# sdrobert/pydrobert-speech

Measured on AMD Instinct MI355X. Metric: frames/s (whole node) + HBM-roofline %, 40-mel fbank 16kHz 25/10ms, higher is better.
Workload: dtype f32

## Files before the change

pydrobert-speech_amd/csrc/pds_internal.h:

```cpp
#pragma once
#include <hip/hip_runtime.h>
#include <stdint.h>

#include <exception>
#include <new>
#include <string>

#include "../../include/pds_amd.h"

namespace pds {

void set_error(const std::string &msg);
int32_t hip_fail(hipError_t err, const char *what);

#define PDS_HIP(call)                                       \
  do {                                                      \
    hipError_t _e = (call);                                 \
    if (_e != hipSuccess) return pds::hip_fail(_e, #call);  \
  } while (0)

struct FastTables {
  int kind = 0;
  int n1 = 0, n2 = 0;
  int rows = 0;
  int num_cus = 0;
  float *d_window = nullptr;
  float *d_twiddle = nullptr;
  float *d_tw_special = nullptr;
  float *d_win_half = nullptr;
  float *d_tw_seed = nullptr;
  float *d_ell_w = nullptr;
  int32_t *d_ell_meta = nullptr;
  int32_t *d_ell_len = nullptr;
  int32_t *d_ell_woff = nullptr;
  int ell_wfloats = 0, ell_slots = 0;
  float *d_seg_w = nullptr;
  int32_t *d_seg_meta = nullptr;
  int seg_rounds = 0, seg_len = 0, seg_wfloats = 0, seg_meta_ints = 0;
  float *d_rs_w = nullptr;
  int32_t *d_rs_meta = nullptr;
  int rs_rounds = 0, rs_len = 0, rs_wfloats = 0;
  float *d_rsn_w = nullptr;
  int32_t *d_rsn_meta = nullptr;
  int rsn_rounds = 0, rsn_len = 0, rsn_wfloats = 0;
  int rs_eslot = -1;
  float *d_ms_w = nullptr;
  int32_t *d_ms_meta = nullptr;
  int ms_rounds = 0, ms_len = 0, ms_wfloats = 0, ms_meta_ints = 0, ms_slots = 0;
  long ms_reads = 0;
  int walk = 0;
  long rs_reads = 0, rs_cost = 0, ell_reads = 0, seg_reads = 0;
  float *d_mf_tab = nullptr;
  int mf_rows = 0;
};

}

struct pds_stft_plan {
  pds_stft_desc d;
  int device = 0;
  int num_bins = 0;
  float *d_window_f32 = nullptr;
  double *d_window_f64 = nullptr;
  int32_t *d_row_ptr = nullptr;
  int32_t *d_col = nullptr;
  float *d_val_f32 = nullptr;
  double *d_val_f64 = nullptr;
  float2 *d_tw_f32 = nullptr;
  double2 *d_tw_f64 = nullptr;
  pds::FastTables fast;
};

namespace pds {
struct SiFftTables {
  int blocks = 0;
  bool big = false;
  float2 *d_spectra = nullptr;
  float2 *d_twiddle = nullptr;
  float2 *d_twiddle2k = nullptr;
  int num_cus = 0;
};
}

struct pds_si_plan {
  pds_si_desc d;
  int device = 0;
  int mpad = 0;
  float *d_taps_f32 = nullptr;
  double *d_taps_f64 = nullptr;
  float *d_window_f32 = nullptr;
  double *d_window_f64 = nullptr;
  pds::SiFftTables fft;
};

namespace pds {

int32_t si_fft_tables_create(pds_si_plan *plan, const double *taps);
void si_fft_tables_destroy(pds_si_plan *plan);
int64_t si_fft_scratch_len(const pds_si_plan *plan, int32_t B, int64_t max_frames);
struct SiFftShape;
SiFftShape si_fft_shape_of(const pds_si_plan *plan, int32_t B, int64_t max_frames);
int32_t launch_si_fft(const pds_si_plan *plan, const float *d_signal, const int64_t *d_offsets,
                      const int64_t *d_lengths, const int64_t *d_nframes, const int64_t *d_row_off,
                      int32_t B, int64_t max_frames, int64_t start, const int64_t *d_starts, float *d_scratch,
                      float *d_out, int64_t out_stride, void *stream);

struct BatchArgs {
  const void *d_signal;
  const int64_t *d_offsets, *d_lengths, *d_nframes, *d_row_off;
  int32_t B;
  int64_t max_frames;
  int32_t pad_left;
  double preemph;
  void *d_out;
  int64_t out_stride;
  hipStream_t stream;
  bool in_f64 = false, out_f64 = false;
  bool in_i16 = false;
  int dl_K = 0;
  double dl_taps[16] = {0};
  int64_t *d_chunk_prefix = nullptr;
  bool stretch = false;
  double *d_stat_part = nullptr;
  int32_t *grid_waves_out = nullptr;
  bool prefix_prepared = false;
};

int32_t launch_stft_generic_f32(const pds_stft_plan *plan, const BatchArgs &a);
int32_t launch_stft_generic_f64(const pds_stft_plan *plan, const BatchArgs &a);
int32_t fast_tables_create(pds_stft_plan *plan, const double *window, const int32_t *row_ptr,
                           const int32_t *col, const double *val);
void fast_tables_destroy(pds_stft_plan *plan);
int32_t launch_stft_fast_f32(const pds_stft_plan *plan, const BatchArgs &a);
void fast_plan_geometry(const pds_stft_plan *plan, int32_t out[3]);
bool fast_has_f64in(const pds_stft_plan *plan);
bool fast_has_fused_deltas(const pds_stft_plan *plan);
bool fast_has_fused_cmvn(const pds_stft_plan *plan);
int32_t launch_chunk_prefix(const int64_t *d_nframes, int B, int groups, int64_t *d_prefix, hipStream_t stream);
int32_t launch_cmvn_rows_partials(const float *d_in, int64_t in_stride, const int64_t *d_row_off, const int64_t *d_nrows,
                                  int32_t B, int32_t C, int32_t norm_var, const int64_t *d_chunk_prefix,
                                  const double *d_partials, int32_t grid_waves, double *d_stats, void *d_out,
                                  int32_t out_is_f64, int64_t out_stride, int32_t *d_zero_var, void *stream);

template <typename F>
int32_t no_throw(const char *what, F &&body) {
  try {
    return body();
  } catch (const std::bad_alloc &) {
    set_error(std::string(what) + ": out of host memory");
    return PDS_ERR_NOMEM;
  } catch (const std::exception &err) {
    set_error(std::string(what) + ": " + err.what());
    return PDS_ERR_INVALID;
  }
}

int32_t check_plan_device(int plan_device, const char *what);

template <typename T>
int32_t upload(T **dst, const T *src, size_t count) {
  *dst = nullptr;
  if (count == 0) return PDS_OK;
  PDS_HIP(hipMalloc((void **)dst, count * sizeof(T)));
  PDS_HIP(hipMemcpy(*dst, src, count * sizeof(T), hipMemcpyHostToDevice));
  return PDS_OK;
}

#ifndef PDS_PREEMPH_FMA
#define PDS_PREEMPH_FMA 1
#endif
__device__ __forceinline__ float preemph_sample(float cur, float prev, float c) {
#if PDS_PREEMPH_FMA
  return fmaf(-c, prev, cur);
#else
  float t;
  asm("v_mul_f32 %0, %1, %2" : "=v"(t) : "v"(c), "v"(prev));
  return cur - t;
#endif
}
__device__ __forceinline__ double preemph_sample(double cur, double prev, double c) {
  double t;
  asm("v_mul_f64 %0, %1, %2" : "=v"(t) : "v"(c), "v"(prev));
  return cur - t;
}

__device__ __forceinline__ int64_t reflect_index(int64_t i, int64_t n) {
  if (i >= 0 && i < n) return i;
  const int64_t period = 2 * n;
  int64_t m = i % period;
  if (m < 0) m += period;
  return m < n ? m : period - 1 - m;
}

}
```

pydrobert-speech_amd/csrc/stft_fast.hip:

```cpp
#include "stft_wave_launch.h"

namespace pds {

#if PDS_STAMPS
unsigned long long *g_stamp_buf = nullptr;
extern "C" __attribute__((visibility("default"))) void pds_debug_set_stamp_buffer(unsigned long long *d_buf) {
  g_stamp_buf = d_buf;
}
#endif

extern "C" __attribute__((visibility("default"))) int32_t pds_build_experiments(void) { return PDS_EXPERIMENTS ? 1 : 0; }

bool fast_has_f64in(const pds_stft_plan *plan) { return plan->fast.kind && fast_f64in_kind(plan->fast.kind); }

static int fast_geometry_rows(const FastTables &ft, int *minw);

bool fast_has_fused_cmvn(const pds_stft_plan *plan) {
  const FastTables &ft = plan->fast;
  int minw = 0;
  if (!ft.kind || ft.n2 != 16 || (ft.n1 != 32 && ft.n1 != 64) || !fast_geometry_rows(ft, &minw)) return false;
  return ft.walk == 1 || ft.walk == 3 || (ft.walk == 2 && minw <= 2);
}

bool fast_has_fused_deltas(const pds_stft_plan *plan) {
  const FastTables &ft = plan->fast;
  return ft.kind && fast_deltas_kind(ft.kind) && ft.rsn_rounds >= 1 && ft.rsn_rounds <= 2 &&
         (!plan->d.include_energy || ft.rs_eslot >= 0);
}

__global__ __launch_bounds__(1024) void chunk_prefix_kernel(const int64_t *nframes, int B, int groups, int64_t *prefix) {
  __shared__ int64_t part[1024];
  const int per = (B + 1023) / 1024, lo = threadIdx.x * per, hi = lo + per < B ? lo + per : B;
  int64_t sum = 0;
  for (int b = lo; b < hi; ++b) sum += (nframes[b] + groups - 1) / groups;
  part[threadIdx.x] = sum;
  __syncthreads();
  for (int step = 1; step < 1024; step <<= 1) {
    const int64_t add = threadIdx.x >= (unsigned)step ? part[threadIdx.x - step] : 0;
    __syncthreads();
    part[threadIdx.x] += add;
    __syncthreads();
  }
  int64_t run = part[threadIdx.x] - sum;
  for (int b = lo; b < hi; ++b) {
    prefix[b] = run;
    run += (nframes[b] + groups - 1) / groups;
  }
  if (threadIdx.x == 1023) prefix[B] = part[1023];
}

int32_t launch_chunk_prefix(const int64_t *d_nframes, int B, int groups, int64_t *d_prefix, hipStream_t stream) {
  hipLaunchKernelGGL(chunk_prefix_kernel, dim3(1), dim3(1024), 0, stream, d_nframes, B, groups, d_prefix);
  PDS_HIP(hipGetLastError());
  return PDS_OK;
}

#define PDS_GEOM(N1, N2, R, MINW) int32_t launch_geom_##N1##_##N2##_##R(const pds_stft_plan *plan, const BatchArgs &a);
#ifdef PDS_DEV_ONLY512
PDS_GEOM(32, 16, 25, 4)
#else
#include "stft_geoms.def"
#endif
#undef PDS_GEOM

static int fast_geometry_rows(const FastTables &ft, int *minw = nullptr) {
  if (!ft.kind) return 0;
#define PDS_GEOM(N1, N2, R, MINW)                          \
  if (ft.n1 == N1 && ft.n2 == N2 && ft.rows <= R) {        \
    if (minw) *minw = MINW;                                \
    return R;                                              \
  }
#ifdef PDS_DEV_ONLY512
  PDS_GEOM(32, 16, 25, 4)
#else
#include "stft_geoms.def"
#endif
#undef PDS_GEOM
  return 0;
}

void fast_plan_geometry(const pds_stft_plan *plan, int32_t out[3]) {
  const FastTables &ft = plan->fast;
  const int rows = fast_geometry_rows(ft);
  out[0] = rows ? ft.n1 : 0;
  out[1] = rows ? ft.n2 : 0;
  out[2] = rows;
}

int32_t launch_stft_fast_f32(const pds_stft_plan *plan, const BatchArgs &a) {
  const FastTables &ft = plan->fast;
  const int rows = fast_geometry_rows(ft);
#define PDS_GEOM(N1, N2, R, MINW) \
  if (ft.n1 == N1 && ft.n2 == N2 && rows == R) return launch_geom_##N1##_##N2##_##R(plan, a);
#ifdef PDS_DEV_ONLY512
  PDS_GEOM(32, 16, 25, 4)
#else
#include "stft_geoms.def"
#endif
#undef PDS_GEOM
  set_error("stft_batch: no fused kernel for this plan");
  return PDS_ERR_INVALID;
}

int32_t fast_tables_create(pds_stft_plan *plan, const double *window, const int32_t *row_ptr,
                           const int32_t *col, const double *val) {
  FastTables &ft = plan->fast;
  ft.kind = 0;
  const pds_stft_desc &d = plan->d;
  int n1 = 0, n2 = 0;
  switch (d.dft_size) {
    case 128: n1 = 16; n2 = 8; break;
    case 256: n1 = 32; n2 = 8; break;
    case 512: n1 = 32; n2 = 16; break;
    case 1024: {
      const char *geom = PDS_EXPERIMENTS ? std::getenv("PDS_N1024_GEOM") : nullptr;
      const bool wide = geom && std::strcmp(geom, "32x32") == 0;
      n1 = wide ? 32 : 64;
      n2 = wide ? 32 : 16;
      break;
    }
    case 2048: n1 = 64; n2 = 32; break;
    case 4096: n1 = 64; n2 = 64; break;
    case 160: n1 = 20; n2 = 8; break;
    case 200: n1 = 25; n2 = 8; break;
    case 240: n1 = 30; n2 = 8; break;
    case 320: n1 = 20; n2 = 16; break;
    case 400: n1 = 25; n2 = 16; break;
    case 480: n1 = 30; n2 = 16; break;
    case 640: n1 = 20; n2 = 32; break;
    case 800: n1 = 25; n2 = 32; break;
    case 960: n1 = 30; n2 = 32; break;
    default: return PDS_OK;
  }
  const bool pow2 = (n1 & (n1 - 1)) == 0;
  if (!pow2 && d.frame_length != d.dft_size) return PDS_OK;
  const char *off = std::getenv("PDS_STFT_GENERIC");
  if (off && off[0] == '1') return PDS_OK;
  if (d.frame_length > d.dft_size || d.frame_length <= d.dft_size / 2) return PDS_OK;
  if (d.frame_shift >= (1 << 22)) return PDS_OK;
  if (d.use_log && !((float)d.log_floor >= 1.17549435e-38f)) return PDS_OK;
  if (d.num_filts > 32767) return PDS_OK;
  const int N = d.dft_size, H1 = n1 / 2, cols = (n1 - 1) / 2 + 1;
  std::vector<float> win((size_t)n1 * n2, 0.0f);
  for (int r = 0; r < n2; ++r)
    for (int k = 0; k < n1; ++k) {
      const int idx = n2 * k + r;
      if (idx < d.frame_length) {
        const float w = (float)window[idx];
        win[(size_t)r * n1 + k] = w == 0.0f ? 0x1p-100f : w;
      }
    }
  std::vector<float> tw((size_t)n2 * cols * 2, 0.0f);
  for (int r = 0; r < n2; ++r)
    for (int k1 = 1; k1 < cols; ++k1) {
      const double ang = -2.0 * M_PI * (double)((r * k1) % N) / (double)N;
      const double scale = (!pow2 || PDS_RDFT_DIT) ? 1.0 : (2 * k1 == H1) ? 1.0 : 0.5;
      tw[((size_t)r * cols + k1) * 2 + 0] = (float)(scale * std::cos(ang));
      tw[((size_t)r * cols + k1) * 2 + 1] = (float)(scale * std::sin(ang));
    }
  std::vector<int32_t> order(d.num_filts);
  for (int f = 0; f < d.num_filts; ++f) order[f] = f;
  auto span = [&](int f) {
    return row_ptr[f + 1] > row_ptr[f] ? col[row_ptr[f + 1] - 1] - (col[row_ptr[f]] & ~3) + 1 : 0;
  };
  std::stable_sort(order.begin(), order.end(), [&](int x, int y) { return span(x) > span(y); });
  const int slots = (d.num_filts + n2 - 1) / n2;
  const int pstr = ((N / 2 + 2 + 15) / 32) * 32 + 16;
  std::vector<int32_t> ell_meta((size_t)std::max(slots, 1) * n2, 0), ell_len(std::max(slots, USLOTS), 0),
      ell_woff(std::max(slots, USLOTS), 0);
  std::vector<float> ell_w;
  for (int sl = 0; sl < slots; ++sl) {
    int longest = 8;
    std::vector<int> first(n2, 0);
    for (int j = 0; j < n2 && sl * n2 + j < d.num_filts; ++j) {
      const int f = order[sl * n2 + j];
      if (row_ptr[f + 1] == row_ptr[f]) continue;
      first[j] = col[row_ptr[f]] & ~3;
      longest = std::max(longest, (span(f) + 7) / 8 * 8);
    }
    {
      std::vector<int> lanes;
      for (int j = 0; j < n2 && sl * n2 + j < d.num_filts; ++j)
        if (span(order[sl * n2 + j]) > 0) lanes.push_back(j);
      std::stable_sort(lanes.begin(), lanes.end(), [&](int x, int y) {
        return span(order[sl * n2 + x]) > span(order[sl * n2 + y]);
      });
      std::vector<std::vector<int>> taken(16);
      for (int j : lanes) {
        const int slack = std::min((longest - span(order[sl * n2 + j])) / 4, first[j] / 4);
        int best_shift = 0, best_cost = 1 << 30;
        for (int sh = 0; sh <= slack; ++sh) {
          const int q = first[j] / 4 - sh;
          int cost = 0;
          for (int other : taken[q % 16]) cost += other != q;
          if (cost < best_cost) {
            best_cost = cost;
            best_shift = sh;
          }
        }
        first[j] -= 4 * best_shift;
        taken[(first[j] / 4) % 16].push_back(first[j] / 4);
      }
    }
    ell_len[sl] = longest;
    ell_woff[sl] = (int32_t)ell_w.size();
    const int wstride = longest + 4;
    ell_w.resize(ell_w.size() + (size_t)n2 * wstride, 0.0f);
    for (int j = 0; j < n2; ++j) {
      const int f = sl * n2 + j < d.num_filts ? order[sl * n2 + j] : -1;
      if (first[j] + longest > pstr)
        first[j] = (pstr - longest) & ~3;
      if (first[j] < 0) return PDS_OK;
      ell_meta[(size_t)sl * n2 + j] = first[j] | ((f + 1) << 16);
      if (f < 0) continue;
      for (int q = row_ptr[f]; q < row_ptr[f + 1]; ++q) {
        const int t = col[q] - first[j];
        if (t < 0 || t >= longest) return PDS_OK;
        ell_w[(size_t)ell_woff[sl] + (size_t)j * wstride + t] = (float)val[q];
      }
    }
  }
  if (ell_w.empty()) ell_w.assign(4, 0.0f);
  ft.ell_wfloats = (int)ell_w.size();
  ft.ell_slots = slots;
  int32_t rc = PDS_OK;
  const int groups = 64 / n2;
  bool dense_bank = false;
  long dense_reads = 0;
  if ((n2 == 16 || (pow2 && n2 >= 32)) && d.num_filts > 0 && d.num_filts <= 65535) {
    long ell_reads = 0;
    for (int sl = 0; sl < slots; ++sl) ell_reads += 2L * (ell_len[sl] / 4);
    ft.ell_reads = ell_reads;
    const int free_slots = (wave_area_floats(n1, n2) - groups * pstr) / groups;
    int best_len = 0, best_rounds = 0;
    long best_reads = 0, any_reads = 0;
    const char *only_len = std::getenv("PDS_SEG_LEN");
    for (int len : {16, 32, 64}) {
      if (only_len && std::atoi(only_len) != len) continue;
      long nseg = 0;
      for (int f = 0; f < d.num_filts; ++f) nseg += (span(f) + len - 1) / len;
      const int rounds = (int)((nseg + 63) / 64);
      if (rounds == 0 || rounds * 64 > 65535) continue;
      int longest = 0;
      for (int f = 0; f < d.num_filts; ++f) longest = std::max(longest, (span(f) + len - 1) / len);
      const long reads = (long)rounds * (len / 4) * (1 + groups) + rounds + (nseg + 63) / 64 + 4 + 4L * ((longest + 3) / 4);
      if (!any_reads || reads < any_reads) any_reads = reads;
      if (rounds * 64 > free_slots) continue;
      if (!best_len || reads < best_reads) best_len = len, best_rounds = rounds, best_reads = reads;
    }
    const char *force = std::getenv("PDS_STFT_SEGMENTED");
    if (!force && std::getenv("PDS_STFT_WALK") && std::strcmp(std::getenv("PDS_STFT_WALK"), "seg") == 0) force = "1";
    auto wanted = [&](long reads) {
      return force      ? force[0] == '1'
             : n2 == 64 ? reads < ell_reads
             : n2 == 32 ? 10 * reads <= 7 * ell_reads
                        : 5 * reads <= 4 * ell_reads || (slots >= 4 && reads < ell_reads);
    };
    const bool want = wanted(best_reads);
    dense_bank = any_reads > 0 && wanted(any_reads);
    dense_reads = any_reads;
    if (best_len && want) {
      const int len = best_len, nslots = best_rounds * 64, wstride = len + 4;
      std::vector<float> seg_w((size_t)nslots * wstride, 0.0f);
      std::vector<int32_t> seg_meta((size_t)nslots + d.num_filts, 0);
      int slot = 0;
      bool ok = true;
      for (int f = 0; f < d.num_filts && ok; ++f) {
        const int count = (span(f) + len - 1) / len;
        seg_meta[(size_t)nslots + f] = slot | (count << 16);
        const int base = count ? col[row_ptr[f]] & ~3 : 0;
        for (int k = 0; k < count; ++k, ++slot) {
          int first = base + k * len;
          if (first + len > pstr) first = (pstr - len) & ~3;
          if (first < 0) ok = false;
          seg_meta[slot] = first;
          for (int q = row_ptr[f]; q < row_ptr[f + 1]; ++q) {
            if (col[q] < base + k * len || col[q] >= base + (k + 1) * len) continue;
            const int t = col[q] - first;
            if (t < 0 || t >= len) ok = false; else seg_w[(size_t)slot * wstride + t] = (float)val[q];
          }
        }
      }
      if (ok) {
        ft.seg_reads = best_reads;
        ft.seg_rounds = best_rounds;
        ft.seg_len = len;
        ft.seg_wfloats = (int)seg_w.size();
        ft.seg_meta_ints = (int)seg_meta.size();
        if (rc == PDS_OK) rc = upload(&ft.d_seg_w, seg_w.data(), seg_w.size());
        if (rc == PDS_OK) rc = upload(&ft.d_seg_meta, seg_meta.data(), seg_meta.size());
      }
    }
  }
  if (n2 == 16 && rc == PDS_OK) {
    RsegTables rs;
    const int area_floats = wave_area_floats(n1, n2);
    if (build_rseg(d.num_filts, row_ptr, col, val, N / 2 + 1, area_floats / 4, 8, rs)) {
      ft.rs_rounds = rs.rounds;
      ft.rs_len = rs.seg_len;
      ft.rs_wfloats = (int)rs.w.size();
      ft.rs_reads = rs.reads_per_lane();
      ft.rs_cost = rs.cost;
      RsegTables rn;
      ft.rs_eslot = -1;
      if (rc == PDS_OK && fast_deltas_kind(N) && build_rseg(d.num_filts, row_ptr, col, val, N / 2 + 1, area_floats / 4, 2, rn, true)) {
        ft.rsn_rounds = rn.rounds;
        ft.rsn_len = rn.seg_len;
        ft.rsn_wfloats = (int)rn.w.size();
        for (size_t at = 0; at < rn.meta.size() && ft.rs_eslot < 0; ++at)
          if ((rn.meta[at] >> 16) == 0) ft.rs_eslot = (int)at;
        rc = upload(&ft.d_rsn_w, rn.w.data(), rn.w.size());
        if (rc == PDS_OK) rc = upload(&ft.d_rsn_meta, rn.meta.data(), rn.meta.size());
      }
      if (rc == PDS_OK) rc = upload(&ft.d_rs_w, rs.w.data(), rs.w.size());
      if (rc == PDS_OK) rc = upload(&ft.d_rs_meta, rs.meta.data(), rs.meta.size());
    }
  }
  if (n2 == 16 && pow2 && rc == PDS_OK && dense_bank) {
    MsegTables ms;
    const int area_floats = wave_area_floats(n1, n2);
    const int max_slots = (area_floats - 4 * pstr) / 16;
    if (build_mseg(d.num_filts, row_ptr, col, val, pstr, max_slots, ms)) {
      ft.ms_rounds = ms.rounds;
      ft.ms_slots = ms.slots;
      ft.ms_len = ms.seg_len;
      ft.ms_wfloats = (int)ms.w.size();
      ft.ms_meta_ints = (int)ms.meta.size();
      ft.ms_reads = ms.reads_per_lane();
      rc = upload(&ft.d_ms_w, ms.w.data(), ms.w.size());
      if (rc == PDS_OK) rc = upload(&ft.d_ms_meta, ms.meta.data(), ms.meta.size());
    }
  }
  {
    const char *force = std::getenv("PDS_STFT_WALK");
    ft.walk = ft.seg_rounds > 0 ? 1 : 0;
    const bool ms_stands_in = ft.walk == 0 && dense_bank && ft.ms_rounds > 0 && N >= PDS_MSEG_MIN_N;
    const long other = ft.walk == 1 ? ft.seg_reads : ms_stands_in ? dense_reads : ft.ell_reads;
    if (ft.rs_rounds > 0 && 10 * ft.rs_reads <= 7 * other) ft.walk = 2;
    if (force && std::strcmp(force, "ell") == 0) ft.walk = 0;
    if (force && std::strcmp(force, "seg") == 0) ft.walk = ft.seg_rounds > 0 ? 1 : 0;
    if (force && std::strcmp(force, "rseg") == 0) ft.walk = ft.rs_rounds > 0 ? 2 : ft.walk;
    if ((ft.walk == 1 || (ft.walk == 0 && ms_stands_in)) && ft.ms_rounds > 0 && N >= PDS_MSEG_MIN_N && !force) ft.walk = 3;
    if (force && std::strcmp(force, "mseg") == 0 && ft.ms_rounds > 0) ft.walk = 3;
    if (std::getenv("PDS_DEBUG_PLAN"))
      std::fprintf(stderr,
                   "pds plan N=%d filters=%d: ell slots %d reads %ld | seg rounds %d len %d reads %ld | rseg rounds %d "
                   "len %d reads %ld cost %ld | mseg rounds %d len %d reads %ld -> walk %d\n",
                   N, d.num_filts, ft.ell_slots, ft.ell_reads, ft.seg_rounds, ft.seg_len, ft.seg_reads, ft.rs_rounds,
                   ft.rs_len, ft.rs_reads, ft.rs_cost, ft.ms_rounds, ft.ms_len, ft.ms_reads, ft.walk);
  }
  if (rc == PDS_OK) rc = upload(&ft.d_ell_w, ell_w.data(), ell_w.size());
  if (rc == PDS_OK) rc = upload(&ft.d_ell_meta, ell_meta.data(), ell_meta.size());
  if (rc == PDS_OK) rc = upload(&ft.d_ell_len, ell_len.data(), ell_len.size());
  if (rc == PDS_OK) rc = upload(&ft.d_ell_woff, ell_woff.data(), ell_woff.size());
  if (rc == PDS_OK) rc = upload(&ft.d_window, win.data(), win.size());
  if (rc == PDS_OK) rc = upload(&ft.d_twiddle, tw.data(), tw.size());
  if (((n1 == 32 || n1 == 64) && n2 == 16) || lean_geometry(n1, n2)) {
    std::vector<float> wh(win), seed((size_t)n2 * 6);
    for (float &v : wh) v *= PDS_RDFT_DIT ? 1.0f : 0.5f;
    const int mult[3] = {1, 4, n1 / 4};
    for (int r = 0; r < n2; ++r)
      for (int j = 0; j < 3; ++j) {
        const double ang = -2.0 * M_PI * (double)((r * mult[j]) % N) / (double)N;
        seed[((size_t)r * 3 + j) * 2 + 0] = (float)std::cos(ang);
        seed[((size_t)r * 3 + j) * 2 + 1] = (float)std::sin(ang);
      }
    if (rc == PDS_OK) rc = upload(&ft.d_win_half, wh.data(), wh.size());
    if (rc == PDS_OK) rc = upload(&ft.d_tw_seed, seed.data(), seed.size());
  }
  std::vector<float> tws((size_t)n2 * 2);
  for (int r = 0; r < n2; ++r) {
    const double ang = -2.0 * M_PI * (double)r / (double)(2 * n2);
    tws[2 * r] = (float)std::cos(ang);
    tws[2 * r + 1] = (float)std::sin(ang);
  }
  if (rc == PDS_OK) rc = upload(&ft.d_tw_special, tws.data(), tws.size());
  {
    const char *front = PDS_EXPERIMENTS ? std::getenv("PDS_STFT_FRONT") : nullptr;
    const int rows = (d.frame_length + n2 - 1) / n2;
    int bucket = 0;
    for (int b : {20, 25, 28, 30, 32})
      if (!bucket && rows <= b) bucket = b;
    MfmaFrontTables mt;
    if (rc == PDS_OK && n1 == 32 && n2 == 16 && bucket && front && std::strcmp(front, "mfma") == 0 &&
        build_mfma_front(n1, bucket, d.frame_length, window, mt)) {
      std::vector<float> image;
      image.reserve(mt.words());
      image.insert(image.end(), mt.win.begin(), mt.win.end());
      for (int32_t v : mt.off) {
        float f;
        std::memcpy(&f, &v, sizeof f);
        image.push_back(f);
      }
      image.insert(image.end(), mt.emask.begin(), mt.emask.end());
      image.insert(image.end(), mt.a_re.begin(), mt.a_re.end());
      image.insert(image.end(), mt.a_im.begin(), mt.a_im.end());
      image.insert(image.end(), mt.tw.begin(), mt.tw.end());
      rc = upload(&ft.d_mf_tab, image.data(), image.size());
      ft.mf_rows = bucket;
    }
  }
  if (rc != PDS_OK) return rc;
  hipDeviceProp_t prop;
  PDS_HIP(hipGetDeviceProperties(&prop, plan->device));
  ft.num_cus = prop.multiProcessorCount;
  ft.n1 = n1;
  ft.n2 = n2;
  ft.rows = (d.frame_length + n2 - 1) / n2;
  ft.kind = d.dft_size;
  return PDS_OK;
}

void fast_tables_destroy(pds_stft_plan *plan) {
  FastTables &ft = plan->fast;
  (void)hipFree(ft.d_window);
  (void)hipFree(ft.d_twiddle);
  (void)hipFree(ft.d_tw_special);
  (void)hipFree(ft.d_win_half);
  (void)hipFree(ft.d_tw_seed);
  (void)hipFree(ft.d_mf_tab);
  (void)hipFree(ft.d_rs_w);
  (void)hipFree(ft.d_ms_w);
  (void)hipFree(ft.d_ms_meta);
  (void)hipFree(ft.d_rsn_w);
  (void)hipFree(ft.d_rsn_meta);
  (void)hipFree(ft.d_rs_meta);
  (void)hipFree(ft.d_seg_w);
  (void)hipFree(ft.d_seg_meta);
  (void)hipFree(ft.d_ell_w);
  (void)hipFree(ft.d_ell_meta);
  (void)hipFree(ft.d_ell_len);
  (void)hipFree(ft.d_ell_woff);
  ft = FastTables();
}

}
```

pydrobert-speech_amd/csrc/stft_wave_kernel.h:

```cpp
#pragma once
#include <algorithm>
#include <atomic>
#include <cmath>
#include <cstdio>
#include <cstdlib>
#include <cstring>
#include <type_traits>
#include <vector>

#include "fft_inlane.h"
#include "mfma_front.h"
#include "rseg_tables.h"
#include "mseg_tables.h"
#include "pds_internal.h"

#include "stft_switches.h"

namespace pds {

__device__ __forceinline__ void keep_alive(float v) { asm volatile("" ::"v"(v)); }

struct FastParams {
  const void *sig;
  const int64_t *offsets, *lengths, *nframes, *row_off;
  void *out;
  int64_t out_stride;
  const float *win_lane;
  const float2 *tw_lane;
  const float2 *tw_special;
  const float *win_half;
  const float2 *tw_seed;
  const float *ell_w;
  const int32_t *ell_meta;
  const int32_t *ell_len;
  const int32_t *ell_woff;
  int ell_wfloats, ell_slots, ell_meta_pad, ell_meta_ints;
  int seg_rounds, seg_len, num_filts;
  int L, S, pad_left, include_energy, use_power, use_log;
  float log_floor, inv_L, preemph;
  double preemph_d;
  int chunks_per_utt, num_utts;
  int waves;
  int area_f;
  unsigned waves_rcp;
  int lds_ticket_off;
  int dyn;
  const float *mf_tab;
  unsigned long long *stamps;
  const int64_t *chunk_prefix;
  double *stat_part;
  int stat_c, stat_cs;
  int lds_stat_off;
  int dl_inner;
  int dl_order;
  int dl_debug;
  int dl_eslot;
  float dl_f1[5], dl_f2[9];
  int step_utts, step_chunks;
};

__device__ __forceinline__ float mul_legacy(float x, float y) {
  float z;
  asm("v_mul_legacy_f32 %0, %1, %2" : "=v"(z) : "v"(x), "v"(y));
  return z;
}

template <int N1>
__device__ __forceinline__ float window_mul(int n1, float x, float w) {
#if PDS_WINDOW_CONTRACT
  return n1 < N1 / 2 ? x * w : mul_legacy(x, w);
#else
  return mul_legacy(x, w);
#endif
}

template <int M>
__device__ __forceinline__ float dpp_row_shr_keep(float old, float src) {
  return __int_as_float(__builtin_amdgcn_update_dpp(__float_as_int(old), __float_as_int(src),
                                                    0x110 + M, 0xf, 0xf, false));
}

__device__ __forceinline__ float fast_log(float x) {
  return __builtin_amdgcn_logf(x) * 0.69314718055994530942f;
}

__device__ __forceinline__ float floor_log(float v, float floor) {
  return fast_log(__builtin_elementwise_maximum(v, floor));
}

typedef int Int4 __attribute__((ext_vector_type(4)));
template <typename T>
__device__ __forceinline__ T load_const(const T *ptr) {
  typedef const T __attribute__((address_space(4))) *const_ptr;
  return *(const_ptr)(uintptr_t)ptr;
}

template <int CTRL>
__device__ __forceinline__ float dpp_add(float x) {
  return x + __int_as_float(__builtin_amdgcn_update_dpp(0, __float_as_int(x), CTRL, 0xf, 0xf, false));
}

__device__ __forceinline__ void wave_sync() {
  __builtin_amdgcn_fence(__ATOMIC_RELEASE, "wavefront");
  __builtin_amdgcn_wave_barrier();
  __builtin_amdgcn_fence(__ATOMIC_ACQUIRE, "wavefront");
}

#ifndef PDS_TWOPASS
#define PDS_TWOPASS 1
#endif
#ifndef PDS_LEAN_2048
#define PDS_LEAN_2048 1
#endif
constexpr bool lean_geometry(int n1, int n2) { return PDS_LEAN_2048 && n1 == 64 && n2 == 32; }
constexpr int wave_area_floats(int n1, int n2) {
  const int cols = (n1 - 1) / 2 + 1, groups = 64 / n2, one_pass = groups * cols * (n2 + 2) * 2;
  return (PDS_TWOPASS && n1 == 64 && n2 == 16) ? 2688 : lean_geometry(n1, n2) ? groups * cols * (n2 + 4) : one_pass;
}
constexpr int win_table_stride(int rows) { return ((rows + 3) & ~3) % 8 == 4 ? ((rows + 3) & ~3) : ((rows + 3) & ~3) + 4; }

template <int N1, int N2, int NROWS>
struct WaveGeom {
  static constexpr int N = N1 * N2;
  static constexpr int NREG = (N1 - 1) / 2;
  static constexpr int COLS = NREG + 1;
  static constexpr int CPL = (COLS + N2 - 1) / N2;
  static constexpr bool FULL = COLS % N2 == 0;
  static constexpr bool DIST = N2 >= 16;
  static constexpr int GROUPS = 64 / N2;
  static constexpr int NB = N / 2 + 1;
  static constexpr int RS = N2 + 2;
  static constexpr bool TWOPASS = PDS_TWOPASS && N1 == 64 && N2 == 16;
  static constexpr bool LEAN = lean_geometry(N1, N2);
  static constexpr int RSF = N2 + 4;
  static constexpr int XROWS = TWOPASS ? N2 : COLS;
  static constexpr int EXCH_F2 = wave_area_floats(N1, N2) / 2;
  static_assert(LEAN ? GROUPS * XROWS * RSF <= EXCH_F2 * 2 : GROUPS * XROWS * RS <= EXCH_F2, "the exchange must fit the wave's area");
  static_assert(!LEAN || (CPL == 1 && N2 >= 32), "lean form: one column per lane");
  static constexpr int PSTR = ((NB + 1 + 15) / 32) * 32 + 16;
  static_assert(GROUPS * PSTR <= EXCH_F2 * 2, "P must fit over the exchange area");
  static constexpr int XMIN_F = LEAN ? GROUPS * XROWS * RSF : GROUPS * XROWS * RS * 2;
  static constexpr int GCH = XMIN_F / 64 < NROWS ? XMIN_F / 64 : NROWS;
  static_assert(N % 2 == 0 && CPL >= 1 && N2 <= 64 && (RS * 8) % 16 == 0, "geometry");
  static_assert(inl::is_pow2(N1) ? (FULL || N2 == 2 * COLS) : 600 % N1 == 0,
                "in-lane DFT sizes: 2^k, or a divisor of 600");
  static_assert(NROWS <= N1 && NROWS > 0, "rows");
};

constexpr int USLOTS = 4;

typedef float f32x4 __attribute__((ext_vector_type(4)));

template <int N1, int N2, int NROWS, int MAXWAVES, int MINW, bool ELL_LDS, bool PRE, int SEG = 0, int MF = 0,
          bool RSG = false, typename TIN = float, typename TOUT = float, int DLT = 0, bool STR = false, bool PF = false>
__global__ __launch_bounds__(MAXWAVES * 64, MINW) void stft_wave_kernel(const FastParams p) {
  static_assert(!PF || (DLT == 0 && !STR && MF == 0 && !PRE && std::is_same<TIN, float>::value && (N1 == 32 || N1 == 64) && N2 == 16),
                "prefetch: 16-lane power-of-two geometries, float32 samples, round-robin scheduling");
  constexpr bool STRETCH = DLT > 0 || STR;
  static_assert(!(STR && DLT > 0), "stretch scheduling is part of the fused-deltas launches already");
  static_assert(DLT == 0 || (DLT == 2 && N2 == 16 && RSG && std::is_same<TOUT, float>::value && MF == 0),
                "fused deltas: row-segment walk, float32 features");
  static_assert(MF == 0 || std::is_same<TIN, float>::value, "matrix-pipe front end: float32 samples");
  static_assert(std::is_same<TIN, float>::value || std::is_same<TIN, double>::value || std::is_same<TIN, int16_t>::value, "samples: float32, float64 or int16");
  using G = WaveGeom<N1, N2, NROWS>;
  constexpr int N = G::N, COLS = G::COLS, NREG = G::NREG, RS = G::RS, NB = G::NB, PSTR = G::PSTR;
  constexpr int MSLOTS = 2 * MF + 1;
  static_assert(MF == 0 || (N2 == 16 && N1 == 32 && MF == mfma_front_steps(NROWS)), "matrix-pipe front end: 32 x 16");
  static_assert(MF == 0 || 4 * MSLOTS * 64 <= G::EXCH_F2 * 2, "edge-frame gather reuses the exchange area");
  constexpr int NBP = (NB + 3) / 4 * 4;
  static_assert(!RSG || (G::GROUPS == 4 && ELL_LDS && !SEG && (NBP + 1) * 4 <= G::EXCH_F2 * 2),
                "row-segment walk: four frames per wave, tables in LDS");
  extern __shared__ __attribute__((aligned(16))) float smem[];
  const int lane = threadIdx.x & 63;
  const int wave = __builtin_amdgcn_readfirstlane(threadIdx.x >> 6);
  const int g = lane / N2, r = lane % N2;
  constexpr bool F64S = std::is_same<TIN, double>::value;
  constexpr bool PAIR = F64S && N2 == 16 && MF == 0;
  const int rho = PAIR ? ((r & 7) * 2 + (r >> 3)) : r;
  constexpr int LOADSPAN = PAIR ? (NROWS + 1) / 2 * 32 : NROWS * N2;
  [[maybe_unused]] const unsigned long long st_entry = PDS_STAMPS ? __builtin_readcyclecounter() : 0;
  float *wbase = smem + wave * p.area_f;
  [[maybe_unused]] double *wstat = reinterpret_cast<double *>(smem + p.lds_stat_off) + wave * (2 * p.stat_cs);
  constexpr bool STATS = STR && G::GROUPS == 4 && (SEG != 0 || (RSG && MINW <= 2));
  [[maybe_unused]] const bool stats_on = STATS && p.stat_part != nullptr;
  [[maybe_unused]] auto stat_add4 = [&](const int col, const float (&v)[4], const int nf) {
    double t1 = 0.0, t2 = 0.0;
#pragma unroll
    for (int q = 0; q < 4; ++q)
      if (q < nf) {
        const double d = (double)v[q];
        t1 += d;
        t2 = fma(d, d, t2);
      }
    wstat[col] += t1;
    wstat[p.stat_cs + col] += t2;
  };
  float2 *exch = reinterpret_cast<float2 *>(wbase) + g * G::XROWS * RS;
  [[maybe_unused]] float *xf = wbase + g * (G::XROWS * G::RSF);
  float *Pg = wbase + g * PSTR;
  const int nthreads = p.waves * 64;
  float2 *sw_lds = reinterpret_cast<float2 *>(smem + p.waves * p.area_f);
  int *meta_lds = reinterpret_cast<int *>(sw_lds + N2);
  float *ellw_lds = reinterpret_cast<float *>(meta_lds + p.ell_meta_pad);
  constexpr bool TWCHAIN = (PF && PDS_PF_TW == 1) || (PAIR && (N1 == 32 || N1 == 64)) || (PDS_DLT_CHAIN && DLT > 0 && N1 == 32 && N2 == 16) || G::LEAN ||
                           (N1 == 64 && N2 == 16 && (SEG == 2 || PDS_LEAN_1024));
  constexpr bool WINLDS = PF && PDS_PF_WIN == 1;
  constexpr bool WINUSE = G::LEAN || (N1 == 64 && N2 == 16 && (SEG == 2 || PDS_LEAN_1024));
  constexpr int WSTR = win_table_stride(NROWS);
  [[maybe_unused]] float *win_lds = ellw_lds + (ELL_LDS ? p.ell_wfloats : 0);
  if constexpr (WINLDS || WINUSE) {
    const float *wsrc = TWCHAIN ? p.win_half : p.win_lane;
    for (int i = threadIdx.x; i < N2 * WSTR; i += p.waves * 64) {
      const int rr = i / WSTR, k = i - rr * WSTR;
      win_lds[i] = k < NROWS ? wsrc[rr * N1 + k] : 0.0f;
    }
  }
  if (threadIdx.x < N2) sw_lds[threadIdx.x] = p.tw_special[threadIdx.x];
  constexpr bool DYN = PDS_DYN && !STRETCH && !PF;
  [[maybe_unused]] int *ticket_lds = reinterpret_cast<int *>(smem + p.lds_ticket_off);
  if constexpr (DYN) {
    if (threadIdx.x == 0) *ticket_lds = p.waves;
  }
  if constexpr (STR && G::GROUPS == 4 && (SEG != 0 || (RSG && MINW <= 2))) {
    if (p.stat_part) {
      double *z = reinterpret_cast<double *>(smem + p.lds_stat_off);
      for (int i = threadIdx.x; i < p.waves * 2 * p.stat_cs; i += p.waves * 64) z[i] = 0.0;
    }
  }
  if constexpr (RSG) {
    int4 *rec_lds = reinterpret_cast<int4 *>(meta_lds);
    for (int i = threadIdx.x; i < p.seg_rounds * 64; i += nthreads) {
      const int m = p.ell_meta[i], f = (m >> 16) - 1;
      rec_lds[i] = make_int4((m & 0x3fff) * 16, __float_as_int((m & (1 << 14)) ? 1.0f : 0.0f),
                             __float_as_int((m & (1 << 15)) ? 1.0f : 0.0f),
                             f >= 0 ? ((p.include_energy ? 1 : 0) + f) * (int)sizeof(TOUT) : -1);
    }
  } else {
    for (int i = threadIdx.x; i < p.ell_meta_pad; i += nthreads)
      meta_lds[i] = i < p.ell_meta_ints ? p.ell_meta[i] : 0;
  }
#if PDS_FAST_PROLOGUE
  static_assert((G::EXCH_F2 * 2) % 4 == 0, "wave areas are zeroed 16 bytes at a time");
  if constexpr (ELL_LDS) {
    const float4 *src4 = reinterpret_cast<const float4 *>(p.ell_w);
    float4 *dst4 = reinterpret_cast<float4 *>(ellw_lds);
    for (int i = threadIdx.x; i < (p.ell_wfloats >> 2); i += nthreads) dst4[i] = src4[i];
  }
  {
    float4 *z4 = reinterpret_cast<float4 *>(smem);
    for (int i = threadIdx.x; i < p.waves * (p.area_f / 4); i += nthreads) z4[i] = make_float4(0.0f, 0.0f, 0.0f, 0.0f);
  }
#else
  if constexpr (ELL_LDS)
    for (int i = threadIdx.x; i < p.ell_wfloats; i += nthreads) ellw_lds[i] = p.ell_w[i];
  for (int i = threadIdx.x; i < p.waves * p.area_f; i += nthreads) smem[i] = 0.0f;
#endif
  __syncthreads();

  [[maybe_unused]] float win[(MF || WINLDS || WINUSE) ? 1 : NROWS];
  [[maybe_unused]] float twr[(MF || TWCHAIN) ? 1 : COLS], twi[(MF || TWCHAIN) ? 1 : COLS];
  [[maybe_unused]] float sd[6] = {0.0f, 0.0f, 0.0f, 0.0f, 0.0f, 0.0f};
  [[maybe_unused]] float mwin[MSLOTS], mare[MF + 1], maim[MF + 1], mtwr[4], mtwi[4];
  [[maybe_unused]] unsigned moff[MSLOTS];
  if constexpr (MF > 0) {
    const float *tab = p.mf_tab;
#pragma unroll
    for (int sl = 0; sl < MSLOTS; ++sl) {
      mwin[sl] = tab[sl * 64 + lane];
      moff[sl] = (unsigned)reinterpret_cast<const int *>(tab)[(MSLOTS + sl) * 64 + lane] * 4u;
    }
#pragma unroll
    for (int t = 0; t <= MF; ++t) {
      mare[t] = tab[(3 * MSLOTS + t) * 64 + lane];
      maim[t] = tab[(3 * MSLOTS + MF + 1 + t) * 64 + lane];
    }
#pragma unroll
    for (int v = 0; v < 4; ++v) {
      const float2 t = reinterpret_cast<const float2 *>(tab + (3 * MSLOTS + 2 * (MF + 1)) * 64)[v * 64 + lane];
      mtwr[v] = t.x;
      mtwi[v] = t.y;
    }
  } else {
    if constexpr (!WINLDS && !WINUSE) {
      const float *wsrc = TWCHAIN ? p.win_half : p.win_lane;
#pragma unroll
      for (int n1 = 0; n1 < NROWS; ++n1) win[n1] = wsrc[rho * N1 + n1];
    }
    if constexpr (TWCHAIN) {
#pragma unroll
      for (int j = 0; j < 3; ++j) {
        const float2 t = p.tw_seed[rho * 3 + j];
        sd[2 * j] = t.x;
        sd[2 * j + 1] = t.y;
      }
    } else {
#pragma unroll
      for (int k1 = 1; k1 <= NREG; ++k1) {
        const float2 t = p.tw_lane[rho * COLS + k1];
        twr[k1] = t.x;
        twi[k1] = t.y;
      }
    }
  }
  [[maybe_unused]] float pfv[PF ? NROWS : 1];
  [[maybe_unused]] float wl[WINLDS ? NROWS : 1];
  [[maybe_unused]] auto read_window = [&]() {
    if constexpr (WINLDS) {
      const float4 *w4 = reinterpret_cast<const float4 *>(win_lds + rho * WSTR);
#pragma unroll
      for (int j = 0; j < (NROWS + 3) / 4; ++j) {
        const float4 w = w4[j];
        const float wv[4] = {w.x, w.y, w.z, w.w};
#pragma unroll
        for (int u = 0; u < 4; ++u)
          if (4 * j + u < NROWS) wl[4 * j + u] = wv[u];
      }
    }
  };
  read_window();
  [[maybe_unused]] bool pf_ready = false;
  [[maybe_unused]] const int pf_lane = __mul24(g, p.S) + r;
  const int L = p.L, S = p.S;
  const bool use_power = p.use_power != 0;
  const int col0 = p.include_energy ? 1 : 0;

  int b = 0;
  int wg = blockIdx.x;
#ifndef PDS_NO_XCD_MAP
  if ((gridDim.x & 7) == 0) wg = (wg & 7) * (gridDim.x >> 3) + (wg >> 3);
#endif
  int chunk = wg * p.waves + wave;
  if constexpr (!STRETCH) {
    while (chunk >= p.chunks_per_utt && b < p.num_utts) {
      chunk -= p.chunks_per_utt;
      ++b;
    }
  }
  [[maybe_unused]] int rnd = 0, rb = 0, rc = wg * p.waves;
  if constexpr (DYN) {
    while (rc >= p.chunks_per_utt && rb < p.num_utts) {
      rc -= p.chunks_per_utt;
      ++rb;
    }
  }
  [[maybe_unused]] auto take_ticket = [&](const int t) {
    const int jn = (int)__umulhi((unsigned)t, p.waves_rcp), o = t - jn * p.waves;
    while (rnd < jn && rb < p.num_utts) {
      rc += p.step_chunks;
      rb += p.step_utts;
      if (rc >= p.chunks_per_utt) {
        rc -= p.chunks_per_utt;
        ++rb;
      }
      ++rnd;
    }
    b = rb;
    chunk = rc + o;
    while (chunk >= p.chunks_per_utt && b < p.num_utts) {
      chunk -= p.chunks_per_utt;
      ++b;
    }
  };
  [[maybe_unused]] int ticket_v = 0;
  [[maybe_unused]] auto fetch_ticket = [&]() {
    if (lane == 0) ticket_v = __hip_atomic_fetch_add(ticket_lds, 1, __ATOMIC_RELAXED, __HIP_MEMORY_SCOPE_WORKGROUP);
  };
  [[maybe_unused]] auto next_item_dyn = [&](int &nfr_, int &n_, int64_t &sig_off_, int64_t &out_row_) {
    const int last_b = b;
    take_ticket(__builtin_amdgcn_readfirstlane(ticket_v));
    const int pb_ = b < p.num_utts ? b : last_b;
    nfr_ = (int)load_const(p.nframes + pb_);
    n_ = (int)load_const(p.lengths + pb_);
    sig_off_ = load_const(p.offsets + pb_);
    out_row_ = load_const(p.row_off + pb_);
  };
  int nfr = 0, n = 0;
  int64_t sig_off = 0, out_row = 0;
  if (!STRETCH && b < p.num_utts) {
    nfr = (int)load_const(p.nframes + b);
    n = (int)load_const(p.lengths + b);
    sig_off = load_const(p.offsets + b);
    out_row = load_const(p.row_off + b);
  }
  constexpr int DR = 2;
  [[maybe_unused]] int left = 0, e_lo = 0, e_hi = 0, c_last = -1;
  [[maybe_unused]] bool piece_open = false, ran = false;
  [[maybe_unused]] float Wp[DR][4], Wc[DR][4], e_keep = 0.0f;
  if constexpr (STRETCH) {
    const int gw = wg * p.waves + wave, GW = (int)gridDim.x * p.waves;
    const int total = (int)load_const(p.chunk_prefix + p.num_utts);
    const int per = total / GW, rem = total - per * GW;
    const int pos = gw * per + (gw < rem ? gw : rem);
    left = per + (gw < rem ? 1 : 0);
    int lo = 0, hi = p.num_utts;
    while (left > 0 && hi - lo > 1) {
      const int mid = (lo + hi) >> 1;
      if ((int)load_const(p.chunk_prefix + mid) <= pos) lo = mid; else hi = mid;
    }
    b = lo;
    e_lo = left > 0 ? pos - (int)load_const(p.chunk_prefix + lo) : 0;
    chunk = 0;
#pragma unroll
    for (int rd = 0; rd < DR; ++rd)
#pragma unroll
      for (int q = 0; q < 4; ++q) Wp[rd][q] = Wc[rd][q] = 0.0f;
  }
  [[maybe_unused]] auto emit_rows = [&](const int ce, const float (&nx)[DR][4]) {
    if (p.dl_debug & 2) return;
    const int C = p.dl_inner;
    const int W = (p.dl_order + 1) * C, WS = (W + 3) & ~3;
    float *stage = wbase;
    wave_sync();
#pragma unroll
    for (int rd = 0; rd < DR; ++rd) {
      if (rd >= p.seg_rounds) break;
      const int cb = reinterpret_cast<const int4 *>(meta_lds)[rd * 64 + lane].w;
      const int col = cb >= 0 ? cb >> 2 : (p.dl_eslot == rd * 64 + lane ? 0 : -1);
      const float v[12] = {Wp[rd][0], Wp[rd][1], Wp[rd][2], Wp[rd][3], Wc[rd][0], Wc[rd][1],
                           Wc[rd][2], Wc[rd][3], nx[rd][0], nx[rd][1], nx[rd][2], nx[rd][3]};
      float *mine = stage + (col >= 0 ? col : 4 * WS + lane);
      const int wrow = col >= 0 ? WS : 0, wk = col >= 0 ? C : 0;
#pragma unroll
      for (int q = 0; q < 4; ++q) {
        float d = p.dl_f1[0] * v[q + 2];
#pragma unroll
        for (int t = 1; t < 5; ++t) d = fmaf(p.dl_f1[t], v[q + 2 + t], d);
        mine[q * wrow] = v[4 + q];
        mine[q * wrow + wk] = d;
        if (p.dl_order == 2) {
          float dd = p.dl_f2[0] * v[q];
#pragma unroll
          for (int t = 1; t < 9; ++t) dd = fmaf(p.dl_f2[t], v[q + t], dd);
          mine[q * wrow + 2 * wk] = dd;
        }
      }
    }
    wave_sync();
    if (!(p.dl_debug & 1)) {
      float *orow = static_cast<float *>(p.out) + (out_row + (int64_t)ce * 4) * p.out_stride;
      const int fh = nfr - ce * 4;
      const int full = W >> 2, tail = W & 3;
      typedef float F4 __attribute__((ext_vector_type(4), aligned(4)));
      if (fh >= 4 && full <= 64) {
        const int l = lane < full ? lane : full - 1;
        float4 val[4];
#pragma unroll
        for (int q = 0; q < 4; ++q) val[q] = *reinterpret_cast<const float4 *>(stage + q * WS + 4 * l);
        if (lane < full) {
#pragma unroll
          for (int q = 0; q < 4; ++q) {
            F4 o = {val[q].x, val[q].y, val[q].z, val[q].w};
            *reinterpret_cast<F4 *>(orow + (int64_t)q * p.out_stride + 4 * l) = o;
          }
        }
      } else {
        for (int l0 = 0; l0 < full; l0 += 64) {
          const int l = l0 + lane;
          if (l < full) {
#pragma unroll 1
            for (int q = 0; q < 4; ++q)
              if (q < fh) {
                const float4 val = *reinterpret_cast<const float4 *>(stage + q * WS + 4 * l);
                F4 o = {val.x, val.y, val.z, val.w};
                *reinterpret_cast<F4 *>(orow + (int64_t)q * p.out_stride + 4 * l) = o;
              }
          }
        }
      }
      if (tail) {
        const int q = tail == 1 ? lane : tail == 2 ? lane >> 1 : (lane * 11) >> 5;
        const int jj = lane - q * tail;
        if (q < fh && q < 4) orow[(int64_t)q * p.out_stride + 4 * full + jj] = stage[q * WS + 4 * full + jj];
      }
    }
    wave_sync();
  };
  [[maybe_unused]] unsigned long long st_acc[8] = {0, 0, 0, 0, 0, 0, 0, 0};
  [[maybe_unused]] unsigned long long st_prev = PDS_STAMPS ? __builtin_readcyclecounter() : 0;
  [[maybe_unused]] const unsigned long long st_loop = st_prev;
  while (STRETCH || b < p.num_utts) {
    if constexpr (STRETCH) {
      if (!piece_open) {
        if (left <= 0) break;
        nfr = (int)load_const(p.nframes + b);
        const int chunks_b = (nfr + G::GROUPS - 1) / G::GROUPS;
        if (e_lo >= chunks_b) {
          ++b;
          e_lo = 0;
          continue;
        }
        n = (int)load_const(p.lengths + b);
        sig_off = load_const(p.offsets + b);
        out_row = load_const(p.row_off + b);
        e_hi = e_lo + left < chunks_b ? e_lo + left : chunks_b;
        c_last = DLT > 0 ? (e_hi < chunks_b ? e_hi : chunks_b - 1) : e_hi - 1;
        chunk = DLT > 0 ? (e_lo > 0 ? e_lo - 1 : 0) : e_lo;
        piece_open = true;
        ran = false;
      }
      if constexpr (STR) {
        if (ran) ++chunk;
        ran = true;
      }
      if (chunk > c_last) {
        if (DLT > 0 && c_last < e_hi) {
          float nx[DR][4];
#pragma unroll
          for (int rd = 0; rd < DR; ++rd)
#pragma unroll
            for (int q = 0; q < 4; ++q) nx[rd][q] = Wc[rd][3];
          emit_rows(c_last, nx);
        }
        if constexpr (STATS) {
          if (stats_on) {
            wave_sync();
            double *dst = p.stat_part + ((int64_t)(wg * p.waves + wave) + b) * (2 * p.stat_c);
            for (int c = lane; c < p.stat_c; c += 64) {
              dst[c] = wstat[c];
              dst[p.stat_c + c] = wstat[p.stat_cs + c];
              wstat[c] = 0.0;
              wstat[p.stat_cs + c] = 0.0;
            }
            wave_sync();
          }
        }
        left -= e_hi - e_lo;
        ++b;
        e_lo = 0;
        piece_open = false;
        continue;
      }
    }
    int nchunk = chunk + p.step_chunks, nb = b + p.step_utts;
    if (nchunk >= p.chunks_per_utt) {
      nchunk -= p.chunks_per_utt;
      ++nb;
    }
    const int pb = nb < p.num_utts ? nb : b;
    const int tb = chunk * G::GROUPS;
    if constexpr (DYN) {
      if (p.dyn) fetch_ticket();
    }
    if (!STRETCH && tb >= nfr) {
      if (DYN && p.dyn) {
        next_item_dyn(nfr, n, sig_off, out_row);
        continue;
      }
      b = nb;
      chunk = nchunk;
      nfr = (int)load_const(p.nframes + pb);
      n = (int)load_const(p.lengths + pb);
      sig_off = load_const(p.offsets + pb);
      out_row = load_const(p.row_off + pb);
      continue;
    }
    PDS_STAMP(7, 0);
    if constexpr (PDS_STAMPS != 0) ++st_acc[6];
    PDS_PHASE(0);
    [[maybe_unused]] int nfr_nx = 0, n_nx = 0;
    [[maybe_unused]] int64_t sig_off_nx = 0, out_row_nx = 0;
    [[maybe_unused]] auto fetch_next_record = [&]() {
      __builtin_amdgcn_sched_barrier(0);
      nfr_nx = (int)load_const(p.nframes + pb);
      n_nx = (int)load_const(p.lengths + pb);
      sig_off_nx = load_const(p.offsets + pb);
      out_row_nx = load_const(p.row_off + pb);
    };
    [[maybe_unused]] auto issue_prefetch = [&]() {
      const int tb2 = nchunk * G::GROUPS, s02 = tb2 * S - p.pad_left;
      pf_ready = nb < p.num_utts && tb2 + G::GROUPS <= nfr_nx && s02 >= 0 && s02 + (G::GROUPS - 1) * S + LOADSPAN <= n_nx;
      const float *base = pf_ready ? static_cast<const float *>(p.sig) + (sig_off_nx + s02) : p.win_lane;
      const float *xp2 = base + (pf_ready ? pf_lane : r);
#pragma unroll
      for (int n1 = 0; n1 < NROWS; ++n1) {
        pfv[n1] = xp2[n1 * N2];
#if PDS_PF_ILV > 0
        __builtin_amdgcn_sched_group_barrier(0x020, 1, 0);
        __builtin_amdgcn_sched_group_barrier(0x002, PDS_PF_ILV, 0);
#endif
      }
    };
    const TIN *x = static_cast<const TIN *>(p.sig) + sig_off;
    const int start0 = tb * S - p.pad_left;
    bool valid = true;
    float energy = 0.0f;
    const float2 sw = sw_lds[r];
    [[maybe_unused]] float even_sum, odd_sum, Ar[COLS], Ai[COLS];
    if constexpr (MF > 0) {
      int fstart[4];
#pragma unroll
      for (int fg = 0; fg < 4; ++fg) fstart[fg] = start0 + fg * S;
      int wmode = 0;
      if (!(tb + 4 <= nfr && start0 >= (PRE ? 1 : 0) && start0 + 3 * S + NROWS * 16 <= n)) {
        valid = tb + g < nfr;
#pragma unroll
        for (int fg = 0; fg < 4; ++fg) {
          const int st = (tb + fg < nfr ? tb + fg : nfr - 1) * S - p.pad_left;
          fstart[fg] = st;
          int mode = (st < (PRE ? 1 : 0) || st + NROWS * 16 > n) ? 1 : 0;
          if (st < -n || st + L > 2 * n) mode = 2;
          wmode = mode > wmode ? mode : wmode;
        }
      }
      float xs[4][MSLOTS];
      if (wmode == 0) {
#pragma unroll
        for (int fg = 0; fg < 4; ++fg) {
          const char *xg = reinterpret_cast<const char *>(reinterpret_cast<const float *>(x) + fstart[fg]);
#pragma unroll
          for (int sl = 0; sl < MSLOTS; ++sl) {
            float v = (PDS_ABLATE & 1) ? (float)(lane + sl) : *reinterpret_cast<const float *>(xg + moff[sl]);
            if constexpr (PRE) v = preemph_sample(v, *reinterpret_cast<const float *>(xg + moff[sl] - 4), p.preemph);
            xs[fg][sl] = v;
          }
        }
      } else {
        float *tmp = wbase;
        const int *offs = reinterpret_cast<const int *>(p.mf_tab) + MSLOTS * 64 + lane;
#pragma unroll 1
        for (int fg = 0; fg < 4; ++fg) {
          const int st = fstart[fg];
#pragma unroll 1
          for (int sl = 0; sl < MSLOTS; ++sl) {
            int i = st + offs[sl * 64];
            if (wmode == 1) {
              i = i < 0 ? -1 - i : (i >= n ? 2 * n - 1 - i : i);
            } else {
              i = (int)reflect_index((int64_t)i, (int64_t)n);
            }
            float v = (float)x[i];
            if (PRE && i > 0) v = preemph_sample(v, (float)x[i - 1], p.preemph);
            tmp[(fg * MSLOTS + sl) * 64 + lane] = v;
          }
        }
        wave_sync();
#pragma unroll
        for (int fg = 0; fg < 4; ++fg)
#pragma unroll
          for (int sl = 0; sl < MSLOTS; ++sl) xs[fg][sl] = tmp[(fg * MSLOTS + sl) * 64 + lane];
        wave_sync();
      }
      if (p.include_energy) {
        const float *em = p.mf_tab + 2 * MSLOTS * 64 + lane;
        float eg[4] = {0.0f, 0.0f, 0.0f, 0.0f};
#pragma unroll
        for (int sl = 0; sl < MSLOTS; ++sl) {
          const float m = em[sl * 64];
#pragma unroll
          for (int fg = 0; fg < 4; ++fg) {
            const float xm = mul_legacy(xs[fg][sl], m);
            eg[fg] = fmaf(xm, xm, eg[fg]);
          }
        }
#pragma unroll
        for (int fg = 0; fg < 4; ++fg) {
          float e = eg[fg];
          e = dpp_add<0xB1>(e);
          e = dpp_add<0x4E>(e);
          e = dpp_add<0x141>(e);
          e = dpp_add<0x140>(e);
          const int ei = __float_as_int(e);
          const float tot = (__int_as_float(__builtin_amdgcn_readlane(ei, 0)) +
                             __int_as_float(__builtin_amdgcn_readlane(ei, 16))) +
                            (__int_as_float(__builtin_amdgcn_readlane(ei, 32)) +
                             __int_as_float(__builtin_amdgcn_readlane(ei, 48)));
          if (g == fg) energy = tot;
        }
      }
      PDS_STAMP(0, 0);
      PDS_STAMP(1, 1);
      PDS_PHASE(4);
      float sv[4][MF], dv[4][MF], cv[4], uv[4];
#pragma unroll
      for (int fg = 0; fg < 4; ++fg) {
        cv[fg] = xs[fg][2 * MF] * mwin[2 * MF];
        float u = cv[fg];
#pragma unroll
        for (int t = 0; t < MF; ++t) {
          const float a = xs[fg][2 * t] * mwin[2 * t];
          sv[fg][t] = fmaf(xs[fg][2 * t + 1], mwin[2 * t + 1], a);
          dv[fg][t] = fmaf(-xs[fg][2 * t + 1], mwin[2 * t + 1], a);
          u += sv[fg][t];
        }
        uv[fg] = u;
      }
      f32x4 accR[4], accI[4];
#pragma unroll
      for (int fg = 0; fg < 4; ++fg) {
        accR[fg] = f32x4{0.0f, 0.0f, 0.0f, 0.0f};
        accI[fg] = f32x4{0.0f, 0.0f, 0.0f, 0.0f};
      }
      if constexpr (!(PDS_ABLATE & 2)) {
#pragma unroll
        for (int t = 0; t < MF; ++t)
#pragma unroll
          for (int fg = 0; fg < 4; ++fg) {
            accR[fg] = __builtin_amdgcn_mfma_f32_16x16x4f32(mare[t], sv[fg][t], accR[fg], 0, 0, 0);
            accI[fg] = __builtin_amdgcn_mfma_f32_16x16x4f32(maim[t], dv[fg][t], accI[fg], 0, 0, 0);
          }
#pragma unroll
        for (int fg = 0; fg < 4; ++fg) {
          accR[fg] = __builtin_amdgcn_mfma_f32_16x16x4f32(mare[MF], cv[fg], accR[fg], 0, 0, 0);
          accI[fg] = __builtin_amdgcn_mfma_f32_16x16x4f32(maim[MF], uv[fg], accI[fg], 0, 0, 0);
        }
      } else {
#pragma unroll
        for (int fg = 0; fg < 4; ++fg) {
          accR[fg] = f32x4{sv[fg][0], sv[fg][1], sv[fg][2], cv[fg]};
          accI[fg] = f32x4{dv[fg][0], dv[fg][1], dv[fg][2], uv[fg]};
        }
      }
      PDS_PHASE(1);
      float2 *mine = reinterpret_cast<float2 *>(wbase) + (4 * g + 1) * RS + r;
      float *row0 = wbase + r;
#pragma unroll
      for (int fg = 0; fg < 4; ++fg) {
#pragma unroll
        for (int v = 0; v < 4; ++v) {
          float2 val;
          val.x = accR[fg][v] * mtwr[v] - accI[fg][v] * mtwi[v];
          val.y = accR[fg][v] * mtwi[v] + accI[fg][v] * mtwr[v];
          if (v < 3 || g != 3) {
            mine[fg * COLS * RS + v * RS] = val;
          } else {
            row0[fg * COLS * RS * 2] = accR[fg][3];
            row0[fg * COLS * RS * 2 + 16] = accI[fg][3];
          }
        }
      }
    } else {
      int start = start0 + __mul24(g, S);
      int wmode = 0;
      if (!(PF && pf_ready) && !(tb + G::GROUPS <= nfr && start0 >= (PRE ? 1 : 0) &&
            start0 + (G::GROUPS - 1) * S + LOADSPAN <= n)) {
        valid = tb + g < nfr;
        start = (valid ? tb + g : nfr - 1) * S - p.pad_left;
        int mode = 0;
        if (start < (PRE ? 1 : 0) || start + LOADSPAN > n) mode = 1;
        if (start < -n || start + L > 2 * n) mode = 2;
        wmode = __builtin_amdgcn_readfirstlane(__any(mode == 2) ? 2 : (__any(mode == 1) ? 1 : 0));
      }

      float a[N1];
      if (PF && pf_ready) {
#pragma unroll
        for (int n1 = 0; n1 < NROWS; ++n1) a[n1] = pfv[n1];
      } else if (wmode == 0) {
        const TIN *xp = x + (start + r);
        if constexpr (PAIR) {
          typedef double D2 __attribute__((ext_vector_type(2), aligned(8)));
          const TIN *xq = x + (start + 2 * r);
          constexpr int NP = (NROWS + 1) / 2;
          D2 w2[NP];
          [[maybe_unused]] double before = 0.0;
#pragma unroll
          for (int j = 0; j < NP; ++j) w2[j] = *reinterpret_cast<const D2 *>(xq + 32 * j);
          if constexpr (PRE) {
            if (r == 0) before = xq[-1];
          }
          [[maybe_unused]] auto dpp64 = [](double old, double src, auto ctrl) {
            const long long o = __double_as_longlong(old), s_ = __double_as_longlong(src);
            const int lo = __builtin_amdgcn_update_dpp((int)o, (int)s_, decltype(ctrl)::value, 0xf, 0xf, false);
            const int hi = __builtin_amdgcn_update_dpp((int)(o >> 32), (int)(s_ >> 32), decltype(ctrl)::value, 0xf, 0xf, false);
            return __longlong_as_double(((long long)hi << 32) | (unsigned)lo);
          };
#pragma unroll
          for (int j = 0; j < NP; ++j) {
            double u = w2[j].x, v = w2[j].y;
            if constexpr (PRE) {
              const double wrap = j == 0 ? before : dpp64(0.0, (double)w2[j > 0 ? j - 1 : 0].y, inl::Int<0x121>{});
              const double pu = dpp64(wrap, (double)w2[j].y, inl::Int<0x111>{});
              v = preemph_sample(w2[j].y, w2[j].x, (TIN)p.preemph_d);
              u = preemph_sample(w2[j].x, pu, (TIN)p.preemph_d);
            }
            const float fu = (float)u, fv = (float)v;
            a[2 * j] = __int_as_float(__builtin_amdgcn_update_dpp(__float_as_int(fu), __float_as_int(fv), 0x128, 0xf, 0xc, false));
            if (2 * j + 1 < NROWS)
              a[2 * j + 1] = __int_as_float(__builtin_amdgcn_update_dpp(__float_as_int(fv), __float_as_int(fu), 0x128, 0xf, 0x3, false));
          }
        } else if constexpr (F64S) {
          constexpr int FB = (PRE && PDS_F64_ROW_BATCH > 0) ? PDS_F64_ROW_BATCH / 2 : NROWS;
#pragma unroll
          for (int n0 = 0; n0 < NROWS; n0 += FB) {
            TIN cur[FB], prev[FB];
#pragma unroll
            for (int i = 0; i < FB; ++i) {
              if (n0 + i < NROWS) {
                cur[i] = xp[(n0 + i) * N2];
                if constexpr (PRE) prev[i] = xp[(n0 + i) * N2 - 1];
              }
            }
            if constexpr (PRE && PDS_F64_ROW_BATCH > 0) __builtin_amdgcn_sched_barrier(0);
#pragma unroll
            for (int i = 0; i < FB; ++i) {
              if (n0 + i < NROWS) {
                TIN v = cur[i];
                if constexpr (PRE) v = preemph_sample(v, prev[i], (TIN)p.preemph_d);
                a[n0 + i] = (float)v;
              }
            }
          }
        } else {
#pragma unroll
        for (int n1 = 0; n1 < NROWS; ++n1) a[n1] = (PDS_ABLATE & 1) ? (float)(lane + n1) : (float)xp[n1 * N2];
        }
        if constexpr (PRE && !F64S) {
          if constexpr (N2 == 16) {
#if PDS_PREEMPH_DPP
            float carry = 0.0f;
            if (r == 0) carry = (float)xp[-1];
            const float negc = -p.preemph;
            inl::static_for<0, NROWS>([&](auto k) {
              constexpr int n1 = NROWS - 1 - decltype(k)::value;
              if constexpr (n1 > 0) {
                if constexpr (std::is_same<TIN, float>::value)
                  asm volatile("v_fmac_f32_dpp %0, %0, %2 row_shr:1 row_mask:0xf bank_mask:0xf\n\t"
                               "v_fmac_f32_dpp %0, %1, %2 row_shl:15 row_mask:0xf bank_mask:0xf"
                               : "+v"(a[n1]) : "v"(a[n1 - 1]), "v"(negc));
                else
                  asm volatile("s_nop 1\n\t"
                               "v_fmac_f32_dpp %0, %0, %2 row_shr:1 row_mask:0xf bank_mask:0xf\n\t"
                               "v_fmac_f32_dpp %0, %1, %2 row_shl:15 row_mask:0xf bank_mask:0xf"
                               : "+v"(a[n1]) : "v"(a[n1 - 1]), "v"(negc));
              } else {
                if constexpr (std::is_same<TIN, float>::value)
                  asm volatile("v_fmac_f32_dpp %0, %0, %1 row_shr:1 row_mask:0xf bank_mask:0xf" : "+v"(a[0]) : "v"(negc));
                else
                  asm volatile("s_nop 1\n\tv_fmac_f32_dpp %0, %0, %1 row_shr:1 row_mask:0xf bank_mask:0xf" : "+v"(a[0]) : "v"(negc));
                a[0] = fmaf(negc, carry, a[0]);
              }
            });
#else
            float carry = 0.0f;
            if (r == 0) carry = (float)xp[-1];
#pragma unroll
            for (int n1 = 0; n1 < NROWS; ++n1) {
              const float rot = __int_as_float(__builtin_amdgcn_update_dpp(
                  0, __float_as_int(a[n1]), 0x121 , 0xf, 0xf, false));
              const float prev = r == 0 ? carry : rot;
              carry = rot;
              a[n1] = preemph_sample(a[n1], prev, p.preemph);
            }
#endif
          } else if constexpr (N2 == 8 && PDS_PREEMPH_DPP && PDS_PREEMPH_DPP8) {
            float carry = 0.0f;
            if (r == 0) carry = (float)xp[-1];
            const float negc = -p.preemph;
            const bool last = r == N2 - 1;
            inl::static_for<0, NROWS>([&](auto k) {
              constexpr int n1 = NROWS - 1 - decltype(k)::value;
              const float b = last ? 0.0f : a[n1];
              if constexpr (n1 > 0) {
                const float c = last ? a[n1 - 1] : 0.0f;
                asm volatile("s_nop 1\n\t"
                             "v_fmac_f32_dpp %0, %1, %3 row_shr:1 row_mask:0xf bank_mask:0xf\n\t"
                             "v_fmac_f32_dpp %0, %2, %3 row_shl:7 row_mask:0xf bank_mask:0xf"
                             : "+v"(a[n1]) : "v"(b), "v"(c), "v"(negc));
              } else {
                asm volatile("s_nop 1\n\tv_fmac_f32_dpp %0, %1, %2 row_shr:1 row_mask:0xf bank_mask:0xf"
                             : "+v"(a[0]) : "v"(b), "v"(negc));
                a[0] = fmaf(negc, carry, a[0]);
              }
            });
          } else {
#pragma unroll
            for (int n1 = 0; n1 < NROWS; ++n1) a[n1] = preemph_sample(a[n1], (float)xp[n1 * N2 - 1], p.preemph);
          }
        }
      } else {
        float *tmp = wbase;
        inl::static_for<0, (NROWS + G::GCH - 1) / G::GCH>([&](auto cc) {
          constexpr int base = decltype(cc)::value * G::GCH;
          constexpr int top = base + G::GCH < NROWS ? base + G::GCH : NROWS;
#pragma unroll 1
          for (int n1 = base; n1 < top; ++n1) {
            const int idx = n1 * N2 + rho;
            float v = 0.0f;
            if (idx < L) {
              int i = start + idx;
              if (wmode == 1) {
                i = i < 0 ? -1 - i : (i >= n ? 2 * n - 1 - i : i);
              } else {
                i = (int)reflect_index((int64_t)i, (int64_t)n);
              }
              if constexpr (!F64S) {
                v = (float)x[i];
                if (PRE && i > 0) v = preemph_sample(v, (float)x[i - 1], p.preemph);
              } else {
                TIN w = x[i];
                if (PRE && i > 0) w = preemph_sample(w, x[i - 1], (TIN)p.preemph_d);
                v = (float)w;
              }
            }
            tmp[(n1 - base) * 64 + lane] = v;
          }
          wave_sync();
#pragma unroll
          for (int n1 = base; n1 < top; ++n1) a[n1] = tmp[(n1 - base) * 64 + lane];
          wave_sync();
        });
      }
      if (p.include_energy) {
        int lim = L - rho;
        asm volatile("" : "+v"(lim));
#pragma unroll
        for (int n1 = 0; n1 < NROWS; ++n1) {
          const float v = (n1 < N1 / 2 || n1 * N2 < lim) ? a[n1] : 0.0f;
          energy = fmaf(v, v, energy);
        }
      }
      PDS_STAMP(0, 0);
      PDS_STAMP(1, 1);
      PDS_PHASE(4);
      if constexpr (WINLDS) {
#pragma unroll
        for (int n1 = 0; n1 < NROWS; ++n1) a[n1] = window_mul<N1>(n1, a[n1], wl[n1]);
      } else if constexpr (WINUSE) {
        const float4 *w4 = reinterpret_cast<const float4 *>(win_lds + rho * WSTR);
#pragma unroll
        for (int j = 0; j < (NROWS + 3) / 4; ++j) {
          const float4 w = w4[j];
          const float wv[4] = {w.x, w.y, w.z, w.w};
#pragma unroll
          for (int u = 0; u < 4; ++u)
            if (4 * j + u < NROWS) a[4 * j + u] = window_mul<N1>(4 * j + u, a[4 * j + u], wv[u]);
        }
      } else {
#pragma unroll
        for (int n1 = 0; n1 < NROWS; ++n1) a[n1] = window_mul<N1>(n1, a[n1], win[n1]);
      }
      if constexpr (PF) fetch_next_record();
#pragma unroll
      for (int n1 = NROWS; n1 < N1; ++n1) a[n1] = 0.0f;

      if constexpr (PDS_ABLATE & 2) {
        even_sum = a[0];
        odd_sum = a[1];
#pragma unroll
        for (int k = 0; k < COLS; ++k) {
          Ar[k] = a[2 * k];
          Ai[k] = a[2 * k + 1];
        }
      } else if constexpr (inl::is_pow2(N1)) {
#if PDS_RDFT_DIT
        inl::rdft_dit<N1>(a, even_sum, odd_sum, Ar, Ai);
#else
        inl::rdft_scaled<N1>(a, even_sum, odd_sum, Ar, Ai);
#endif
      } else {
        inl::rdft_direct<N1>(a, even_sum, odd_sum, Ar, Ai);
      }

      PDS_PHASE(1);
      if constexpr (G::LEAN) {
        const int slot = (rho & 1) ? N2 + (rho & 3) : (rho >> 1);
        xf[slot] = even_sum;
        xf[(rho & 1) ? N2 + (rho & 3) : N2 / 2 + (rho >> 1)] = odd_sum;
      } else {
        float *row0 = reinterpret_cast<float *>(exch);
        row0[rho] = even_sum;
        row0[N2 + rho] = odd_sum;
      }
      [[maybe_unused]] float ctr[TWCHAIN ? COLS : 1], cti[TWCHAIN ? COLS : 1];
      if constexpr (TWCHAIN) {
#pragma unroll
        for (int j = 0; j < 6; ++j) asm volatile("" : "+v"(sd[j]));
        inl::twiddle_chain<NREG, !PDS_RDFT_DIT>(sd[0], sd[1], sd[2], sd[3], sd[4], sd[5], ctr, cti);
      }
#pragma unroll
      for (int k1 = 1; k1 <= NREG; ++k1) {
        const float wr_ = TWCHAIN ? ctr[TWCHAIN ? k1 : 0] : twr[TWCHAIN ? 0 : k1];
        const float wi_ = TWCHAIN ? cti[TWCHAIN ? k1 : 0] : twi[TWCHAIN ? 0 : k1];
        float2 v;
        v.x = Ar[k1] * wr_ - Ai[k1] * wi_;
        v.y = Ar[k1] * wi_ + Ai[k1] * wr_;
        if constexpr ((PDS_ABLATE & 4) != 0) {
          Ar[k1] = v.x;
          Ai[k1] = v.y;
        } else if (G::TWOPASS && k1 >= N2) {
          Ar[k1] = v.x;
          Ai[k1] = v.y;
        } else if constexpr (G::LEAN) {
          xf[k1 * G::RSF + rho] = v.x;
          Ai[k1] = v.y;
        } else {
          exch[k1 * RS + rho] = v;
        }
      }
    }
    PDS_STAMP(2, 0);
    wave_sync();

    float pw[G::CPL][N2 + 1];
    float sp0 = 0.0f, sp1 = 0.0f;
    constexpr bool PSPLIT = PDS_PAIR_SPLIT && N2 == 2 * COLS && (N2 == 64 || N2 == 32);
    constexpr int PH = N2 / 2, PQ = N2 / 4;
    [[maybe_unused]] const int ph = r / (N2 / 2), pc = r % (N2 / 2);
    if constexpr (PSPLIT) {
      static_assert(!PSPLIT || (G::CPL == 1 && COLS == PH), "pair split: the columns fill half the frame's lanes");
      const float4 *row = reinterpret_cast<const float4 *>(exch + pc * RS);
      float zr[PH], zi[PH], Hr[PH], Hi[PH];
#pragma unroll
      for (int j = 0; j < PH; ++j) {
        const float4 v = row[j];
        zr[j] = ph ? v.z : v.x;
        zi[j] = ph ? v.w : v.y;
      }
      PDS_PHASE(5);
      inl::CFFT<PH, 1>::run(zr, zi, Hr, Hi);
      PDS_PHASE(2);
      inl::static_for<0, PQ>([&](auto k_) {
        constexpr int k = decltype(k_)::value;
        float ar, br, ai, bi;
        if constexpr (N2 == 64) {
          const auto sr_ = __builtin_amdgcn_permlane32_swap(__float_as_uint(Hr[k]), __float_as_uint(Hr[k + PQ]), false, false);
          const auto si_ = __builtin_amdgcn_permlane32_swap(__float_as_uint(Hi[k]), __float_as_uint(Hi[k + PQ]), false, false);
          ar = __uint_as_float(sr_[0]), br = __uint_as_float(sr_[1]);
          ai = __uint_as_float(si_[0]), bi = __uint_as_float(si_[1]);
        } else {
          const auto sr_ = __builtin_amdgcn_permlane16_swap(__float_as_uint(Hr[k]), __float_as_uint(Hr[k + PQ]), false, false);
          const auto si_ = __builtin_amdgcn_permlane16_swap(__float_as_uint(Hi[k]), __float_as_uint(Hi[k + PQ]), false, false);
          ar = __uint_as_float(sr_[0]), br = __uint_as_float(sr_[1]);
          ai = __uint_as_float(si_[0]), bi = __uint_as_float(si_[1]);
        }
        float ur, ui;
        inl::mul_tw<N2, k>(br, bi, ur, ui);
        const float tr = ph ? ui : ur, ti = ph ? -ur : ui;
        const float yar = ar + tr, yai = ai + ti, ybr = ar - tr, ybi = ai - ti;
        pw[0][k] = yar * yar + yai * yai;
        pw[0][PQ + k] = ybr * ybr + ybi * ybi;
        if (pc == 0) {
          exch[k + PQ * ph] = make_float2(yar, yai);
          exch[k + PQ * ph + PH] = make_float2(ybr, ybi);
        }
      });
#pragma unroll
      for (int k2 = PH; k2 <= N2; ++k2) pw[0][k2] = 0.0f;
      wave_sync();
      {
        const float2 ya = exch[r], yb = exch[(N2 - r) & (N2 - 1)];
        const float ar = ya.x, ai = ya.y, br = yb.x, bi = yb.y;
        const float sr = ar + br, si = ai - bi;
        const float dr = ar - br, di = ai + bi;
        const float tr = sw.x * di + sw.y * dr;
        const float ti = sw.y * di - sw.x * dr;
        const float xr = sr + tr, xi = si + ti;
        const float yr = sr - tr, yi = ti - si;
        sp0 = 0.25f * (xr * xr + xi * xi);
        sp1 = 0.25f * (yr * yr + yi * yi);
      }
    } else
#pragma unroll
    for (int q = 0; q < G::CPL; ++q) {
      const int kk = q * N2 + r;
      if constexpr (G::TWOPASS) {
        if (q > 0) {
          wave_sync();
#pragma unroll
          for (int k1 = q * N2; k1 < (q + 1) * N2 && k1 <= NREG; ++k1) exch[(k1 - q * N2) * RS + rho] = make_float2(Ar[k1], Ai[k1]);
          wave_sync();
        }
      }
      const float4 *row = reinterpret_cast<const float4 *>(exch + (G::TWOPASS ? r : kk) * RS);
      float zr[N2], zi[N2], Yr[N2], Yi[N2];
      if constexpr (G::LEAN) {
        const float4 *rowf = reinterpret_cast<const float4 *>(xf + r * G::RSF);
#pragma unroll
        for (int j = 0; j < N2 / 4; ++j) {
          const float4 v = rowf[j];
          zr[4 * j] = v.x, zr[4 * j + 1] = v.y, zr[4 * j + 2] = v.z, zr[4 * j + 3] = v.w;
        }
        wave_sync();
        {
          const int slot = (rho & 1) ? (rho >> 1) : N2 + (rho & 3);
          xf[slot] = even_sum;
          xf[(rho & 1) ? N2 / 2 + (rho >> 1) : N2 + (rho & 3)] = odd_sum;
        }
#pragma unroll
        for (int k1 = 1; k1 <= NREG; ++k1) xf[k1 * G::RSF + rho] = Ai[k1];
        wave_sync();
#pragma unroll
        for (int j = 0; j < N2 / 4; ++j) {
          const float4 v = rowf[j];
          zi[4 * j] = v.x, zi[4 * j + 1] = v.y, zi[4 * j + 2] = v.z, zi[4 * j + 3] = v.w;
        }
      } else
#pragma unroll
      for (int j = 0; j < N2 / 2; ++j) {
        float4 v;
        if constexpr (PDS_ABLATE & 4) {
          v = make_float4(Ar[(2 * j) % COLS], Ai[(2 * j) % COLS], Ar[(2 * j + 1) % COLS], Ai[(2 * j + 1) % COLS]);
        } else {
          v = row[j];
        }
        zr[2 * j] = v.x;
        zi[2 * j] = v.y;
        zr[2 * j + 1] = v.z;
        zi[2 * j + 1] = v.w;
      }
      if constexpr (PF && PDS_PF_PLACE == 0) {
        PDS_PHASE(5);
#if PDS_PF_ILV > 0
        __builtin_amdgcn_sched_group_barrier(0x100, N2 / 2, 0);
#endif
        if (q == 0) issue_prefetch();
      }
      if constexpr (PDS_ABLATE & 8) {
#pragma unroll
        for (int k2 = 0; k2 < N2; ++k2) {
          Yr[k2] = zr[k2];
          Yi[k2] = zi[k2];
        }
      } else {
        if constexpr (!(PF && PDS_PF_PLACE == 0)) PDS_PHASE(5);
        inl::CFFT<N2, 1>::run(zr, zi, Yr, Yi);
        if (q + 1 < G::CPL) {
          PDS_PHASE(1);
        } else {
          PDS_PHASE(2);
        }
      }
#pragma unroll
      for (int k2 = 0; k2 < N2; ++k2) pw[q][k2] = Yr[k2] * Yr[k2] + Yi[k2] * Yi[k2];
      pw[q][N2] = 0.0f;
      if constexpr (!G::DIST) {
        if (q == 0 && r == 0)
          inl::rdft_finish_power<2 * N2>(Yr, Yi, [&](auto mm, float re, float im) {
            pw[q][decltype(mm)::value] = re * re + im * im;
          });
      } else if (q == 0) {
        float ar, ai, br, bi;
        if constexpr (N2 == 16 && !PDS_PACKED_LDS) {
          ar = Yr[0], ai = Yi[0], br = Yr[0], bi = Yi[0];
          inl::static_for<1, N2 / 2 + 1>([&](auto mm) {
            constexpr int m = decltype(mm)::value;
            ar = dpp_row_shr_keep<m>(ar, Yr[m]);
            ai = dpp_row_shr_keep<m>(ai, Yi[m]);
            br = dpp_row_shr_keep<m>(br, Yr[N2 - m]);
            bi = dpp_row_shr_keep<m>(bi, Yi[N2 - m]);
          });
        } else {
          float2 *hand = G::LEAN ? reinterpret_cast<float2 *>(xf) : exch;
          if (r == 0) {
            if constexpr (N2 % 2 == 0) {
              float4 *hand4 = reinterpret_cast<float4 *>(hand);
#pragma unroll
              for (int k2 = 0; k2 < N2; k2 += 2) hand4[k2 / 2] = make_float4(Yr[k2], Yi[k2], Yr[k2 + 1], Yi[k2 + 1]);
            } else {
#pragma unroll
              for (int k2 = 0; k2 < N2; ++k2) hand[k2] = make_float2(Yr[k2], Yi[k2]);
            }
          }
          wave_sync();
          const float2 ya = hand[r], yb = hand[(N2 - r) & (N2 - 1)];
          ar = ya.x, ai = ya.y, br = yb.x, bi = yb.y;
        }
        const float sr = ar + br, si = ai - bi;
        const float dr = ar - br, di = ai + bi;
        const float tr = sw.x * di + sw.y * dr;
        const float ti = sw.y * di - sw.x * dr;
        const float xr = sr + tr, xi = si + ti;
        const float yr = sr - tr, yi = ti - si;
        sp0 = (TWCHAIN && !PDS_RDFT_DIT ? 1.0f : 0.25f) * (xr * xr + xi * xi);
        sp1 = (TWCHAIN && !PDS_RDFT_DIT ? 1.0f : 0.25f) * (yr * yr + yi * yi);
      }
    }
    if (!use_power) {
#pragma unroll
      for (int q = 0; q < G::CPL; ++q)
#pragma unroll
        for (int k2 = 0; k2 <= N2; ++k2) pw[q][k2] = __builtin_amdgcn_sqrtf(pw[q][k2]);
      sp0 = __builtin_amdgcn_sqrtf(sp0);
      sp1 = __builtin_amdgcn_sqrtf(sp1);
    }
    Int4 lens4 = {0, 0, 0, 0}, woff4 = {0, 0, 0, 0};
    if constexpr (!RSG && !SEG) {
      lens4 = load_const(reinterpret_cast<const Int4 *>(p.ell_len));
      woff4 = load_const(reinterpret_cast<const Int4 *>(p.ell_woff));
    }
    const int slot_len[USLOTS] = {lens4.x, lens4.y, lens4.z, lens4.w};
    const int slot_woff[USLOTS] = {woff4.x, woff4.y, woff4.z, woff4.w};
    static_assert(USLOTS == 4, "slot tables are fetched as one int4 each");
    PDS_STAMP(3, 0);
    wave_sync();
    float *const Pw = RSG ? wbase + g : Pg;
    constexpr int PB = RSG ? 4 : 1;
    constexpr int PDUMP = RSG ? NBP : PSTR - 1;
    if constexpr (PSPLIT) {
      const int lo_bin = pc + N1 * PQ * ph, hi_bin = N / 2 - pc - N1 * PQ * ph;
      float *const Plo = Pw + lo_bin * PB, *const Phi = Pw + (hi_bin - N1 * (PQ - 1)) * PB;
#pragma unroll
      for (int k = 0; k < PQ; ++k) {
        Plo[N1 * k * PB] = pw[0][k];
        Phi[N1 * (PQ - 1 - k) * PB] = pw[0][PQ + k];
      }
    } else
#pragma unroll
    for (int q = 0; q < G::CPL; ++q) {
      const int kk = q * N2 + r;
      if (!G::DIST && q == 0 && r == 0) {
#pragma unroll
        for (int m = 0; m <= N2; m += (N1 % 2 ? 2 : 1)) Pw[(m * N1 / 2) * PB] = pw[q][m];
      } else {
        const bool live = G::FULL || kk < COLS;
        if constexpr (G::FULL && PDS_MIRROR_REBASE) {
          float *const Pa = Pw + kk * PB, *const Pm = Pw + (N1 - kk) * PB;
#pragma unroll
          for (int k2 = 0; k2 < N2 / 2; ++k2) Pa[N1 * k2 * PB] = pw[q][k2];
#pragma unroll
          for (int k2 = N2 / 2; k2 < N2; ++k2) Pm[N1 * (N2 - 1 - k2) * PB] = pw[q][k2];
        } else
#pragma unroll
        for (int k2 = 0; k2 < N2; ++k2) {
          const int bin = (k2 < N2 / 2) ? kk + N1 * k2 : N - kk - N1 * k2;
          Pw[(live ? bin : PDUMP) * PB] = pw[q][k2];
        }
      }
    }
    if constexpr (G::DIST) {
      const bool has = r <= N2 / 2 && (N1 % 2 == 0 || r % 2 == 0);
      Pw[(has ? r * N1 / 2 : PDUMP) * PB] = sp0;
      Pw[(has ? (N2 - r) * N1 / 2 : PDUMP) * PB] = sp1;
    }
    if constexpr (RSG) {
      constexpr int PADF = (NBP - NB) * 4;
      wbase[NB * 4 + (lane < PADF ? lane : PADF - 1)] = 0.0f;
    } else {
#pragma unroll
      for (int j0 = 0; j0 < PSTR - NB; j0 += N2) {
        const int j = j0 + r;
        Pg[NB + (j < PSTR - NB ? j : PSTR - NB - 1)] = 0.0f;
      }
    }
    TOUT *obase = static_cast<TOUT *>(p.out) + (out_row + tb) * p.out_stride;
    const unsigned lane_off = (unsigned)(g * (int)p.out_stride + col0);
    if (p.include_energy) {
      if constexpr (MF == 0) {
        energy = dpp_add<0xB1>(energy);
        energy = dpp_add<0x4E>(energy);
        energy = dpp_add<0x141>(energy);
        if constexpr (N2 >= 16) energy = dpp_add<0x140>(energy);
        if constexpr (N2 >= 32) energy += __shfl_xor(energy, 16, 64);
        if constexpr (N2 == 64) energy += __shfl_xor(energy, 32, 64);
      }
      float e = energy * p.inv_L;
      if (!use_power) e = __builtin_amdgcn_sqrtf(e);
      if (p.use_log) e = floor_log(e, p.log_floor);
      if (DLT == 0 && valid && r == 0) {
        unsigned off = (lane_off - col0) * (unsigned)sizeof(TOUT);
        asm("" : "+v"(off));
        *reinterpret_cast<TOUT *>(reinterpret_cast<char *>(obase) + off) = (TOUT)e;
      }
      if constexpr (DLT > 0) e_keep = e;
      if constexpr (STATS) {
        if (stats_on) {
          const float e4[4] = {__int_as_float(__builtin_amdgcn_readlane(__float_as_int(e), 0)),
                               __int_as_float(__builtin_amdgcn_readlane(__float_as_int(e), 16)),
                               __int_as_float(__builtin_amdgcn_readlane(__float_as_int(e), 32)),
                               __int_as_float(__builtin_amdgcn_readlane(__float_as_int(e), 48))};
          if (lane == 0) stat_add4(0, e4, nfr - tb);
        }
      }
    }
    PDS_STAMP(4, 0);
    PDS_PHASE(3);
    int metas[USLOTS] = {0};
    if constexpr (!RSG && !SEG) {
#pragma unroll
      for (int sl = 0; sl < USLOTS; ++sl) metas[sl] = meta_lds[sl * N2 + r];
    }
    wave_sync();
    [[maybe_unused]] const int frames_here = nfr - tb;
    if constexpr (STRETCH) {
    } else if constexpr (PF) {
      b = nb;
      chunk = nchunk;
      nfr = nfr_nx;
      n = n_nx;
      sig_off = sig_off_nx;
      out_row = out_row_nx;
      if constexpr (PDS_PF_PLACE == 1) issue_prefetch();
    } else if (DYN && p.dyn) {
      next_item_dyn(nfr, n, sig_off, out_row);
    } else {
      b = nb;
      chunk = nchunk;
      nfr = (int)load_const(p.nframes + pb);
      n = (int)load_const(p.lengths + pb);
      sig_off = load_const(p.offsets + pb);
      out_row = load_const(p.row_off + pb);
    }

    auto run_slot = [&](const int meta, const int len, const int slot_woff_) {
      const float4 *prow = reinterpret_cast<const float4 *>(Pg + (meta & 0xffff));
      const int woff = slot_woff_ + __mul24(r, len + 4);
      float acc0 = 0.0f, acc1 = 0.0f, acc2 = 0.0f, acc3 = 0.0f;
      const float4 *wrow = reinterpret_cast<const float4 *>((ELL_LDS ? ellw_lds : p.ell_w) + woff);
      auto step = [&]() {
        const float4 w0 = wrow[0];
        const float4 p0 = prow[0];
        __builtin_amdgcn_sched_group_barrier(0x100, 2, 0);
        const float4 w1 = wrow[1];
        const float4 p1 = prow[1];
        __builtin_amdgcn_sched_group_barrier(0x100, 2, 0);
        acc0 = fmaf(w0.x, p0.x, acc0);
        acc1 = fmaf(w0.y, p0.y, acc1);
        acc2 = fmaf(w0.z, p0.z, acc2);
        acc3 = fmaf(w0.w, p0.w, acc3);
        acc0 = fmaf(w1.x, p1.x, acc0);
        acc1 = fmaf(w1.y, p1.y, acc1);
        acc2 = fmaf(w1.z, p1.z, acc2);
        acc3 = fmaf(w1.w, p1.w, acc3);
        wrow += 2;
        prow += 2;
      };
      const unsigned steps = (PDS_ABLATE & 32) ? 1u : (unsigned)len >> 3;
      if constexpr (N >= PDS_ELL_DEEP_N) {
#pragma unroll 1
        for (unsigned i = steps >> 2; i != 0; --i) {
          step();
          step();
          step();
          step();
        }
        if (steps & 2u) {
          step();
          step();
        }
      } else {
#pragma unroll 1
        for (unsigned i = steps >> 1; i != 0; --i) {
          step();
          step();
        }
      }
      if (steps & 1u) step();
      float acc = (acc0 + acc1) + (acc2 + acc3);
      if (p.use_log) acc = floor_log(acc, p.log_floor);
      if constexpr (PDS_ABLATE & 64) {
        keep_alive(acc);
      } else {
        const unsigned byte_off = (lane_off + (unsigned)(meta >> 16) - 1u) * (unsigned)sizeof(TOUT);
        if (valid && meta >= 0x10000)
          *reinterpret_cast<TOUT *>(reinterpret_cast<char *>(obase) + byte_off) = (TOUT)acc;
      }
    };
    if constexpr (RSG) {
      const float4 *P4 = reinterpret_cast<const float4 *>(wbase);
      const int t4n = p.seg_len >> 2;
      char *const orow0 = reinterpret_cast<char *>(obase);
      const int64_t row_bytes = p.out_stride * (int64_t)sizeof(TOUT);
      auto round_body = [&](const int rd, float (&logged)[4]) {
        const int4 rec = reinterpret_cast<const int4 *>(meta_lds)[rd * 64 + lane];
        const float4 *prow = reinterpret_cast<const float4 *>(reinterpret_cast<const char *>(P4) + rec.x);
        const float4 *wrow = reinterpret_cast<const float4 *>(ellw_lds) + __mul24(rd, t4n) * 64 + lane;
        float a0 = 0.0f, a1 = 0.0f, a2 = 0.0f, a3 = 0.0f;
        auto quad = [&](int t4) {
          const float4 w = wrow[t4 * 64];
          const float4 x0 = prow[4 * t4], x1 = prow[4 * t4 + 1], x2 = prow[4 * t4 + 2], x3 = prow[4 * t4 + 3];
          a0 = fmaf(w.x, x0.x, a0);
          a1 = fmaf(w.x, x0.y, a1);
          a2 = fmaf(w.x, x0.z, a2);
          a3 = fmaf(w.x, x0.w, a3);
          a0 = fmaf(w.y, x1.x, a0);
          a1 = fmaf(w.y, x1.y, a1);
          a2 = fmaf(w.y, x1.z, a2);
          a3 = fmaf(w.y, x1.w, a3);
          a0 = fmaf(w.z, x2.x, a0);
          a1 = fmaf(w.z, x2.y, a1);
          a2 = fmaf(w.z, x2.z, a2);
          a3 = fmaf(w.z, x2.w, a3);
          a0 = fmaf(w.w, x3.x, a0);
          a1 = fmaf(w.w, x3.y, a1);
          a2 = fmaf(w.w, x3.z, a2);
          a3 = fmaf(w.w, x3.w, a3);
        };
        if (t4n == 3) {
          quad(0);
          quad(1);
          quad(2);
        } else if (t4n == 1) {
          quad(0);
        } else if (t4n == 2) {
          quad(0);
          quad(1);
        } else {
#pragma unroll 2
          for (int t4 = 0; t4 < t4n; ++t4) quad(t4);
        }
#if PDS_PF_WINAT == 0
        read_window();
#endif
        const float m1 = __int_as_float(rec.y), m2 = __int_as_float(rec.z);
        auto shl = [](float v, auto ctrl) {
          return __int_as_float(__builtin_amdgcn_update_dpp(0, __float_as_int(v), decltype(ctrl)::value, 0xf, 0xf, true));
        };
#if PDS_WALK_DPP_FMAC
        (void)shl;
        asm volatile("s_nop 1\n\t"
                     "v_fmac_f32_dpp %0, %0, %4 row_shl:1 row_mask:0xf bank_mask:0xf bound_ctrl:0\n\t"
                     "v_fmac_f32_dpp %1, %1, %4 row_shl:1 row_mask:0xf bank_mask:0xf bound_ctrl:0\n\t"
                     "v_fmac_f32_dpp %2, %2, %4 row_shl:1 row_mask:0xf bank_mask:0xf bound_ctrl:0\n\t"
                     "v_fmac_f32_dpp %3, %3, %4 row_shl:1 row_mask:0xf bank_mask:0xf bound_ctrl:0\n\t"
                     "v_fmac_f32_dpp %0, %0, %5 row_shl:2 row_mask:0xf bank_mask:0xf bound_ctrl:0\n\t"
                     "v_fmac_f32_dpp %1, %1, %5 row_shl:2 row_mask:0xf bank_mask:0xf bound_ctrl:0\n\t"
                     "v_fmac_f32_dpp %2, %2, %5 row_shl:2 row_mask:0xf bank_mask:0xf bound_ctrl:0\n\t"
                     "v_fmac_f32_dpp %3, %3, %5 row_shl:2 row_mask:0xf bank_mask:0xf bound_ctrl:0"
                     : "+v"(a0), "+v"(a1), "+v"(a2), "+v"(a3) : "v"(m1), "v"(m2));
#else
        a0 = fmaf(shl(a0, inl::Int<0x101>{}), m1, a0);
        a1 = fmaf(shl(a1, inl::Int<0x101>{}), m1, a1);
        a2 = fmaf(shl(a2, inl::Int<0x101>{}), m1, a2);
        a3 = fmaf(shl(a3, inl::Int<0x101>{}), m1, a3);
        a0 = fmaf(shl(a0, inl::Int<0x102>{}), m2, a0);
        a1 = fmaf(shl(a1, inl::Int<0x102>{}), m2, a1);
        a2 = fmaf(shl(a2, inl::Int<0x102>{}), m2, a2);
        a3 = fmaf(shl(a3, inl::Int<0x102>{}), m2, a3);
#endif
        const int coff = rec.w;
        const float vals[4] = {a0, a1, a2, a3};
        unsigned off = (unsigned)coff;
        auto put = [&](const int gg, const float v) {
          if (DLT == 0 && coff >= 0 && gg < frames_here) {
            asm("" : "+v"(off));
            *reinterpret_cast<TOUT *>(orow0 + gg * row_bytes + off) = (TOUT)v;
          }
          logged[gg] = v;
        };
        if (p.use_log) {
#pragma unroll
          for (int gg = 0; gg < 4; ++gg) put(gg, floor_log(vals[gg], p.log_floor));
        } else {
#pragma unroll
          for (int gg = 0; gg < 4; ++gg) put(gg, vals[gg]);
        }
        if constexpr (STATS) {
          if (stats_on && coff >= 0) stat_add4(coff / (int)sizeof(TOUT), logged, frames_here);
        }
      };
      if constexpr (DLT == 0) {
        float unused[4];
        for (int rd = 0; rd < p.seg_rounds; ++rd) round_body(rd, unused);
#if PDS_PF_WINAT == 1
        read_window();
#endif
      } else {
        float cur[DR][4];
#pragma unroll
        for (int rd = 0; rd < DR; ++rd) {
#pragma unroll
          for (int q = 0; q < 4; ++q) cur[rd][q] = 0.0f;
          if (rd < p.seg_rounds) round_body(rd, cur[rd]);
          if (p.dl_eslot == rd * 64 + lane) {
#pragma unroll
            for (int q = 0; q < 4; ++q)
              cur[rd][q] = __int_as_float(__builtin_amdgcn_readlane(__float_as_int(e_keep), 16 * q));
          }
        }
        if (chunk == 0) {
#pragma unroll
          for (int rd = 0; rd < DR; ++rd)
#pragma unroll
            for (int q = 0; q < 4; ++q) Wc[rd][q] = cur[rd][0];
        }
        if (chunk > e_lo) emit_rows(chunk - 1, cur);
#pragma unroll
        for (int rd = 0; rd < DR; ++rd)
#pragma unroll
          for (int q = 0; q < 4; ++q) {
            Wp[rd][q] = Wc[rd][q];
            Wc[rd][q] = cur[rd][q];
          }
        ++chunk;
      }
      PDS_STAMP(5, 0);
      wave_sync();
      continue;
    }
    if constexpr (SEG) {
      static_assert(!SEG || ELL_LDS, "segmented walks: tables in LDS");
      static_assert(SEG != 2 || G::GROUPS == 4, "matrix-pipe segment walk: four frames per wave");
      {
        float4 *part = reinterpret_cast<float4 *>(wbase + G::GROUPS * PSTR);
        constexpr int SEG_DEPTH = N >= PDS_SEG_DEEP_N ? 4 : 2;
        const int steps = p.seg_len >> 2;
        if constexpr (SEG == 2) {
          const int blk = lane >> 2, fr = lane & 3;
          const float *Pj = wbase + fr * PSTR;
          float *pf = reinterpret_cast<float *>(part) + fr;
          const float4 *wbase4 = reinterpret_cast<const float4 *>(ellw_lds) + lane;
          const int last = p.seg_rounds - 1;
          auto meta_of = [&](int rd) { return meta_lds[(rd < last ? rd : last) * 16 + blk]; };
          auto walk = [&](auto steps_c) {
            constexpr int ST = decltype(steps_c)::value;
            f32x4 acc0 = {0.0f, 0.0f, 0.0f, 0.0f}, acc1 = {0.0f, 0.0f, 0.0f, 0.0f};
            auto fetch = [&](float4 (&w)[ST], float4 (&x)[ST], const int rd, const int meta) {
              const float4 *wrow = wbase4 + __mul24(rd, ST) * 64;
              const float4 *prow = reinterpret_cast<const float4 *>(Pj + (meta & 0x7fff));
#pragma unroll
              for (int u = 0; u < ST; ++u) {
                w[u] = wrow[u * 64];
                x[u] = prow[u];
              }
            };
            auto compute = [&](const float4 (&w)[ST], const float4 (&x)[ST], const int meta) {
#pragma unroll
              for (int u = 0; u < ST; ++u) {
                acc0 = __builtin_amdgcn_mfma_f32_4x4x1f32(w[u].x, x[u].x, acc0, 0, 0, 0);
                acc1 = __builtin_amdgcn_mfma_f32_4x4x1f32(w[u].y, x[u].y, acc1, 0, 0, 0);
                acc0 = __builtin_amdgcn_mfma_f32_4x4x1f32(w[u].z, x[u].z, acc0, 0, 0, 0);
                acc1 = __builtin_amdgcn_mfma_f32_4x4x1f32(w[u].w, x[u].w, acc1, 0, 0, 0);
              }
              if (meta & 0x8000) {
                float *dst = pf + (meta >> 16) * 16;
                dst[0] = acc0[0] + acc1[0];
                dst[4] = acc0[1] + acc1[1];
                dst[8] = acc0[2] + acc1[2];
                dst[12] = acc0[3] + acc1[3];
                acc0 = f32x4{0.0f, 0.0f, 0.0f, 0.0f};
                acc1 = f32x4{0.0f, 0.0f, 0.0f, 0.0f};
              }
            };
            if constexpr (ST == 4 && MINW <= 2) {
              float4 wa[ST], xa[ST], wb[ST], xb[ST];
              int ma = meta_of(0), mb = meta_of(1), mc = meta_of(2);
              fetch(wa, xa, 0, ma);
#pragma unroll 1
              for (int rd = 0; rd <= last; rd += 2) {
                const int md = meta_of(rd + 3), me = meta_of(rd + 4);
                if (rd < last) fetch(wb, xb, rd + 1, mb);
                compute(wa, xa, ma);
                if (rd >= last) break;
                if (rd + 1 < last) fetch(wa, xa, rd + 2, mc);
                compute(wb, xb, mb);
                ma = mc;
                mb = md;
                mc = me;
              }
            } else {
              int m = meta_of(0);
#pragma unroll 1
              for (int rd = 0; rd <= last; ++rd) {
                const int next = meta_of(rd + 1);
                float4 w[ST], x[ST];
                fetch(w, x, rd, m);
                compute(w, x, m);
                m = next;
              }
            }
          };
          if (steps == 4) {
            walk(inl::Int<4>{});
          } else {
            walk(inl::Int<8>{});
          }
        } else
        for (int q = 0; q < p.seg_rounds; ++q) {
          const int slot = q * 64 + lane;
          const int first = meta_lds[slot];
          const float4 *wrow = reinterpret_cast<const float4 *>(ellw_lds + __mul24(slot, p.seg_len + 4));
          const float4 *pg[G::GROUPS];
          float acc[G::GROUPS];
#pragma unroll
          for (int gg = 0; gg < G::GROUPS; ++gg) {
            pg[gg] = reinterpret_cast<const float4 *>(wbase + gg * PSTR + first);
            acc[gg] = 0.0f;
          }
#pragma unroll SEG_DEPTH
          for (int i = 0; i < steps; ++i) {
            const float4 w = wrow[i];
            float4 x[G::GROUPS];
#pragma unroll
            for (int gg = 0; gg < G::GROUPS; ++gg) x[gg] = pg[gg][i];
#pragma unroll
            for (int gg = 0; gg < G::GROUPS; ++gg) acc[gg] = fmaf(w.x, x[gg].x, acc[gg]);
#pragma unroll
            for (int gg = 0; gg < G::GROUPS; ++gg) acc[gg] = fmaf(w.y, x[gg].y, acc[gg]);
#pragma unroll
            for (int gg = 0; gg < G::GROUPS; ++gg) acc[gg] = fmaf(w.z, x[gg].z, acc[gg]);
#pragma unroll
            for (int gg = 0; gg < G::GROUPS; ++gg) acc[gg] = fmaf(w.w, x[gg].w, acc[gg]);
          }
          float *dst = reinterpret_cast<float *>(part) + slot * G::GROUPS;
#pragma unroll
          for (int gg = 0; gg < G::GROUPS; ++gg) dst[gg] = acc[gg];
        }
        if constexpr (PDS_STAMPS > 2) PDS_STAMP(4, 0);
        wave_sync();
        const int *fmeta = meta_lds + p.seg_rounds * (SEG == 2 ? 16 : 64);
        constexpr int PSTEP = SEG == 2 ? 4 : 1;
        for (int f = lane; f < p.num_filts; f += 64) {
          const int fm = fmeta[f];
          const float *src = reinterpret_cast<const float *>(part) + (fm & 0xffff) * G::GROUPS;
          float sum[G::GROUPS];
#pragma unroll
          for (int gg = 0; gg < G::GROUPS; ++gg) sum[gg] = 0.0f;
          if constexpr (PDS_MSEG_RED4) {
            const int cnt = fm >> 16;
            for (int k = 0; k < cnt; k += 4) {
              float v[4][G::GROUPS];
#pragma unroll
              for (int u = 0; u < 4; ++u) {
                const float *at = src + G::GROUPS * PSTEP * (k + u < cnt ? k + u : cnt - 1);
                if constexpr (G::GROUPS == 4) {
                  const float4 t = *reinterpret_cast<const float4 *>(at);
                  v[u][0] = t.x, v[u][1] = t.y, v[u][2] = t.z, v[u][3] = t.w;
                } else if constexpr (G::GROUPS == 2) {
                  const float2 t = *reinterpret_cast<const float2 *>(at);
                  v[u][0] = t.x, v[u][1] = t.y;
                } else {
#pragma unroll
                  for (int gg = 0; gg < G::GROUPS; ++gg) v[u][gg] = at[gg];
                }
              }
#pragma unroll
              for (int u = 0; u < 4; ++u) {
                const bool live = k + u < cnt;
#pragma unroll
                for (int gg = 0; gg < G::GROUPS; ++gg) sum[gg] += live ? v[u][gg] : 0.0f;
              }
            }
          } else
          for (int k = fm >> 16; k > 0; --k) {
#pragma unroll
            for (int gg = 0; gg < G::GROUPS; ++gg) sum[gg] += src[gg];
            src += PSTEP * G::GROUPS;
          }
#pragma unroll
          for (int gg = 0; gg < G::GROUPS; ++gg) {
            float v = sum[gg];
            if (p.use_log) v = floor_log(v, p.log_floor);
            if (gg < frames_here) obase[(int64_t)gg * p.out_stride + col0 + f] = (TOUT)v;
            sum[gg] = v;
          }
          if constexpr (STATS) {
            if (stats_on) stat_add4(col0 + f, sum, frames_here);
          }
        }
        PDS_STAMP(5, 0);
        wave_sync();
        continue;
      }
    }
#pragma unroll
    for (int sl = 0; sl < USLOTS; ++sl)
      if (sl < p.ell_slots) run_slot(metas[sl], slot_len[sl], slot_woff[sl]);
    for (int sl = USLOTS; sl < p.ell_slots; ++sl)
      run_slot(meta_lds[sl * N2 + r], load_const(p.ell_len + sl), load_const(p.ell_woff + sl));
    PDS_STAMP(5, 0);
    wave_sync();
  }
  if constexpr (PDS_STAMPS) {
    if (p.stamps && lane == 0) {
      unsigned long long *dst = p.stamps + ((size_t)blockIdx.x * p.waves + wave) * 12;
#pragma unroll
      for (int i = 0; i < 8; ++i) dst[i] = st_acc[i];
      dst[8] = st_entry;
      dst[9] = st_loop;
      dst[10] = __builtin_readcyclecounter();
    }
  }
}

}
```

pydrobert-speech_amd/csrc/stft_wave_launch.h:

```cpp
#pragma once
#include "stft_wave_kernel.h"

namespace pds {


constexpr bool fast_f64in_kind(int n) { return n == 256 || n == 512 || n == 1024 || n == 2048; }

constexpr bool fast_deltas_kind(int n) { return n == 512 || n == 1024; }


template <int N1, int N2, int NROWS, int MINW>
int32_t launch_wave(const pds_stft_plan *plan, const BatchArgs &a) {
  using G = WaveGeom<N1, N2, NROWS>;
#ifndef PDS_DLT_MINW
#define PDS_DLT_MINW 3
#endif
  constexpr int DMINW = (N1 == 64 && N2 == 16) ? 2 : MINW > PDS_DLT_MINW ? PDS_DLT_MINW : MINW;
  constexpr int CU_WAVES_STFT = 4 * MINW;
  constexpr int F64_MINW = (N1 == 64 && N2 == 16) ? 2 : MINW, F64_WAVES = 4 * F64_MINW;
  const int CU_WAVES = a.dl_K > 0 ? 4 * DMINW : a.in_f64 ? F64_WAVES : CU_WAVES_STFT;
  const FastTables &ft = plan->fast;
  FastParams p;
  p.sig = a.d_signal;
  p.offsets = a.d_offsets;
  p.lengths = a.d_lengths;
  p.nframes = a.d_nframes;
  p.row_off = a.d_row_off;
  p.out = a.d_out;
  p.out_stride = a.out_stride;
  p.win_lane = ft.d_window;
  p.tw_lane = (const float2 *)ft.d_twiddle;
  p.tw_special = (const float2 *)ft.d_tw_special;
  constexpr bool LEAN_ALL = G::LEAN || (PDS_LEAN_1024 && N1 == 64 && N2 == 16);
  p.win_half = LEAN_ALL ? ft.d_win_half : nullptr;
  p.tw_seed = LEAN_ALL ? (const float2 *)ft.d_tw_seed : nullptr;
  p.ell_w = ft.d_ell_w;
  p.ell_meta = ft.d_ell_meta;
  p.ell_len = ft.d_ell_len;
  p.ell_woff = ft.d_ell_woff;
  p.ell_wfloats = ft.ell_wfloats;
  p.ell_slots = ft.ell_slots;
  p.L = plan->d.frame_length;
  p.S = plan->d.frame_shift;
  p.pad_left = a.pad_left;
  p.include_energy = plan->d.include_energy;
  p.use_power = plan->d.use_power;
  p.use_log = plan->d.use_log;
  p.log_floor = (float)plan->d.log_floor;
  p.inv_L = 1.0f / (float)plan->d.frame_length;
  p.num_utts = a.B;
  const int64_t chunks = (a.max_frames + G::GROUPS - 1) / G::GROUPS;
  if (chunks * a.B > 0x7fffffff || chunks > 0x3fffffff || a.out_stride * G::GROUPS > (a.out_f64 ? 0x0fffffff : 0x1fffffff) ||
      a.max_frames * plan->d.frame_shift > 0x7fffffff) {
    set_error("stft_batch: too many frame chunks in one call");
    return PDS_ERR_INVALID;
  }
  p.chunks_per_utt = (int)chunks;
  const size_t lds_cu = 160 * 1024;
  const size_t per_wave = (size_t)G::EXCH_F2 * 8;
  const int stat_c = a.d_stat_part ? plan->d.num_filts + (plan->d.include_energy ? 1 : 0) : 0;
  const int stat_cs = (stat_c + 3) & ~3;
  const size_t stat_pw = (size_t)2 * stat_cs * 8;
  int shapes[4][2] = {{CU_WAVES / 2, 2}, {CU_WAVES, 1}, {CU_WAVES * 3 / 4, 1}, {CU_WAVES * 5 / 8, 1}};
#ifdef PDS_ONE_WG
  shapes[0][0] = CU_WAVES, shapes[0][1] = 1;
#endif
  if (CU_WAVES % 8 != 0) {
    shapes[0][0] = CU_WAVES, shapes[0][1] = 1;
    shapes[1][0] = CU_WAVES * 2 / 3, shapes[1][1] = 1;
    shapes[2][0] = CU_WAVES / 3, shapes[2][1] = 1;
    shapes[3][0] = CU_WAVES / 3, shapes[3][1] = 1;
  }
  constexpr int CU_WAVES_K = CU_WAVES_STFT;
  int waves = CU_WAVES / 2, wgs_per_cu = 2;
  size_t area_bytes = per_wave;
  bool in_lds = false;
  p.seg_rounds = 0;
  p.seg_len = 0;
  p.num_filts = plan->d.num_filts;
  const bool pre = a.preemph != 0.0;
  int walk = 0;
  const bool dl = a.dl_K > 0 && ft.rsn_rounds > 0;
  constexpr bool PFG = (N1 == 32 || N1 == 64) && N2 == 16;
  const char *pf_env = std::getenv("PDS_STFT_PF");
  constexpr bool PF_PRODUCT = N1 == 64 && N2 == 16;
  [[maybe_unused]] constexpr bool PF_MSEG = false;
  constexpr bool MSEG3 = N1 == 64 && N2 == 16;
  constexpr int MS_WAVES = MSEG3 ? 12 : 4 * MINW, MS_MINW = MSEG3 ? 3 : MINW;
  static_assert(!MSEG3 || !PDS_LEAN_1024 || MINW == 3, "the 64 x 16 geometry is instantiated for three waves per SIMD (stft_geoms.def)");
  const bool pf_ok = (PDS_EXPERIMENTS || PF_PRODUCT) && PFG && !pre && !a.in_f64 && !a.in_i16 && !a.stretch && a.dl_K == 0 &&
                     ft.d_win_half && ft.d_tw_seed && !(pf_env && pf_env[0] == '0');
  constexpr int PF_WSTR = ((NROWS + 3) & ~3) % 8 == 4 ? ((NROWS + 3) & ~3) : ((NROWS + 3) & ~3) + 4;
  const size_t pf_extra = (PDS_PF_WIN == 1) ? (size_t)N2 * PF_WSTR * 4 : 0;
  const size_t lean_extra = LEAN_ALL ? (size_t)N2 * win_table_stride(NROWS) * 4 : 0;
  const size_t mseg3_extra = LEAN_ALL ? 0 : (size_t)N2 * win_table_stride(NROWS) * 4;
  constexpr bool MSG = G::GROUPS == 4 && inl::is_pow2(N1);
  constexpr bool SEGOK = G::GROUPS == 4 || (inl::is_pow2(N1) && N2 >= 32);
  for (int cand = (G::GROUPS == 4) ? (dl ? 2 : ft.walk) : (SEGOK && ft.walk == 1 ? 1 : 0); cand >= 0 && !in_lds; --cand) {
    if (cand == 3 && (!MSG || ft.ms_rounds == 0 || pre || a.in_f64 || a.in_i16)) continue;
    if ((cand == 2 && !dl && ft.rs_rounds == 0) || (cand == 1 && (ft.seg_rounds == 0 || pre || a.in_f64 || a.in_i16))) continue;
    const int meta_ints = cand == 3 ? ft.ms_meta_ints : cand == 2 ? (dl ? ft.rsn_rounds : ft.rs_rounds) * 64 : cand == 1 ? ft.seg_meta_ints : ft.ell_slots * N2;
    const int meta_pad = cand == 2 ? meta_ints * 4 : (std::max(meta_ints, USLOTS * N2) + 3) / 4 * 4;
    const size_t fixed = (size_t)N2 * 8 + (size_t)meta_pad * 4 + (cand == 2 && pf_ok ? pf_extra : 0) + lean_extra +
                         (cand == 3 && MSEG3 ? mseg3_extra : 0);
    const size_t table_bytes = (size_t)(cand == 3 ? ft.ms_wfloats : cand == 2 ? (dl ? ft.rsn_wfloats : ft.rs_wfloats) : cand == 1 ? ft.seg_wfloats : ft.ell_wfloats) * 4;
    if (cand == 1 && (size_t)G::GROUPS * G::PSTR * 4 + (size_t)ft.seg_rounds * 64 * 4 * G::GROUPS > per_wave) continue;
    if (cand == 3 && (size_t)G::GROUPS * G::PSTR * 4 + (size_t)ft.ms_slots * 64 > per_wave) continue;
    const size_t area_c = (cand == 3 && MSEG3)
                              ? std::max((size_t)G::XMIN_F * 4, (size_t)G::GROUPS * G::PSTR * 4 + (size_t)ft.ms_slots * 64)
                              : per_wave;
    const int ms_shapes[5][2] = {{12, 1}, {11, 1}, {10, 1}, {9, 1}, {8, 1}};
    const int (*try_shapes)[2] = (cand == 3 && MSEG3) ? ms_shapes : shapes;
    for (int si = 0; si < ((cand == 3 && MSEG3) ? 5 : 4); ++si) {
      const int *shape = try_shapes[si];
      if (shape[0] * (area_c + stat_pw) + fixed + table_bytes + 48 <= lds_cu / shape[1]) {
        waves = shape[0];
        wgs_per_cu = shape[1];
        in_lds = true;
        area_bytes = area_c;
        break;
      }
    }
    p.ell_meta_pad = meta_pad;
    p.ell_meta_ints = meta_ints;
    if (in_lds && cand == 3) {
      p.ell_w = ft.d_ms_w;
      p.ell_meta = ft.d_ms_meta;
      p.ell_wfloats = ft.ms_wfloats;
      p.seg_rounds = ft.ms_rounds;
      p.seg_len = ft.ms_len;
    } else if (in_lds && cand == 1) {
      p.ell_w = ft.d_seg_w;
      p.ell_meta = ft.d_seg_meta;
      p.ell_wfloats = ft.seg_wfloats;
      p.seg_rounds = ft.seg_rounds;
      p.seg_len = ft.seg_len;
    } else if (in_lds && cand == 2) {
      p.ell_w = dl ? ft.d_rsn_w : ft.d_rs_w;
      p.ell_meta = dl ? ft.d_rsn_meta : ft.d_rs_meta;
      p.ell_wfloats = dl ? ft.rsn_wfloats : ft.rs_wfloats;
      p.seg_rounds = dl ? ft.rsn_rounds : ft.rs_rounds;
      p.seg_len = dl ? ft.rsn_len : ft.rs_len;
    }
    if (in_lds) walk = cand;
  }
#ifdef PDS_FORCE_WAVES
  if (in_lds && PDS_FORCE_WAVES <= CU_WAVES / 2) waves = PDS_FORCE_WAVES, wgs_per_cu = 2;
#endif
  const size_t fixed = (size_t)N2 * 8 + (size_t)p.ell_meta_pad * 4 + (walk == 2 && in_lds && pf_ok ? pf_extra : 0) + lean_extra +
                       (walk == 3 && in_lds && MSEG3 ? mseg3_extra : 0);
  const size_t table_bytes = (size_t)p.ell_wfloats * 4;
  if (a.in_i16 && !in_lds) {
    set_error("stft_batch_i16in: not served for this plan (filter table outside LDS)");
    return PDS_ERR_INVALID;
  }
  if (pre && !in_lds) {
    if (a.in_f64 || a.out_f64 || a.dl_K > 0 || a.d_stat_part) {
      set_error("stft_batch: fused pre-emphasis with the filter table outside LDS is served for float32 samples and plain "
                "float32 features only");
      return PDS_ERR_INVALID;
    }
    return launch_stft_generic_f32(plan, a);
  }
  p.preemph = (float)a.preemph;
  p.preemph_d = a.preemph;
  p.waves = waves;
  p.mf_tab = ft.d_mf_tab;
#if PDS_STAMPS
  p.stamps = g_stamp_buf;
#else
  p.stamps = nullptr;
#endif
  p.area_f = (int)(area_bytes / 4);
  size_t smem = waves * area_bytes + fixed + (in_lds ? table_bytes : 0);
  smem = (smem + 15) & ~(size_t)15;
  p.lds_ticket_off = (int)(smem / 4);
  smem += 16;
  p.lds_stat_off = (int)(smem / 4);
  smem += (size_t)waves * stat_pw;
  p.stat_part = nullptr;
  p.stat_c = stat_c;
  p.stat_cs = stat_cs;
  p.waves_rcp = (unsigned)((0x100000000ull + (unsigned)waves - 1) / (unsigned)waves);
  {
    const char *dyn_env = std::getenv("PDS_STFT_DYN");
    p.dyn = (dyn_env && dyn_env[0] == '0') ? 0 : 1;
  }
  constexpr bool W4 = G::GROUPS == 4;
  const bool seg = SEGOK && (walk == 1 || walk == 3), rsg = W4 && walk == 2, mseg = MSG && walk == 3;
  auto kern = pre      ? (rsg ? stft_wave_kernel<N1, N2, NROWS, CU_WAVES_K, MINW, true, true, false, 0, W4>
                              : stft_wave_kernel<N1, N2, NROWS, CU_WAVES_K, MINW, true, true>)
              : rsg    ? stft_wave_kernel<N1, N2, NROWS, CU_WAVES_K, MINW, true, false, false, 0, W4>
              : mseg   ? stft_wave_kernel<N1, N2, NROWS, MS_WAVES, MS_MINW, true, false, MSG ? 2 : 0>
              : seg    ? stft_wave_kernel<N1, N2, NROWS, CU_WAVES_K, MINW, true, false, SEGOK ? 1 : 0>
              : in_lds ? stft_wave_kernel<N1, N2, NROWS, CU_WAVES_K, MINW, true, false>
                       : stft_wave_kernel<N1, N2, NROWS, CU_WAVES_K, MINW, false, false>;
  constexpr int MFS = (PDS_EXPERIMENTS && N1 == 32 && N2 == 16) ? mfma_front_steps(NROWS) : 0;
  bool mf = false;
  if constexpr (MFS > 0) {
    if (in_lds && ft.d_mf_tab && ft.mf_rows == NROWS && !mseg) {
      mf = true;
      kern = pre   ? (rsg ? stft_wave_kernel<N1, N2, NROWS, CU_WAVES_K, MINW, true, true, false, MFS, W4>
                          : stft_wave_kernel<N1, N2, NROWS, CU_WAVES_K, MINW, true, true, false, MFS>)
             : rsg ? stft_wave_kernel<N1, N2, NROWS, CU_WAVES_K, MINW, true, false, false, MFS, W4>
             : seg ? stft_wave_kernel<N1, N2, NROWS, CU_WAVES_K, MINW, true, false, W4, MFS>
                   : stft_wave_kernel<N1, N2, NROWS, CU_WAVES_K, MINW, true, false, false, MFS>;
    }
  }
  bool pf_used = false;
  if (MSEG3 && mseg) {
    p.win_half = ft.d_win_half;
    p.tw_seed = (const float2 *)ft.d_tw_seed;
  }
#if PDS_EXPERIMENTS
  if constexpr (PFG) {
    if (pf_ok && in_lds && !mf && (rsg || seg || (mseg && !PF_MSEG))) {
      pf_used = true;
      kern = rsg    ? stft_wave_kernel<N1, N2, NROWS, CU_WAVES_K, MINW, true, false, 0, 0, W4, float, float, 0, false, PFG>
             : mseg ? stft_wave_kernel<N1, N2, NROWS, CU_WAVES_K, MINW, true, false, MSG ? 2 : 0, 0, false, float, float, 0, false, PFG>
                    : stft_wave_kernel<N1, N2, NROWS, CU_WAVES_K, MINW, true, false, SEGOK ? 1 : 0, 0, false, float, float, 0, false, PFG>;
      p.win_half = ft.d_win_half;
      p.tw_seed = (const float2 *)ft.d_tw_seed;
    }
  }
#endif
  bool str_used = false;
  if constexpr (inl::is_pow2(N1))
  if (a.stretch && !pre && !a.in_f64 && !a.in_i16 && a.dl_K == 0 && !mf && a.d_chunk_prefix && in_lds) {
    str_used = true;
    kern = rsg      ? stft_wave_kernel<N1, N2, NROWS, CU_WAVES_K, MINW, true, false, 0, 0, W4, float, float, 0, true>
           : mseg   ? stft_wave_kernel<N1, N2, NROWS, MS_WAVES, MS_MINW, true, false, MSG ? 2 : 0, 0, false, float, float, 0, true>
           : seg    ? stft_wave_kernel<N1, N2, NROWS, CU_WAVES_K, MINW, true, false, SEGOK ? 1 : 0, 0, false, float, float, 0, true>
                    : stft_wave_kernel<N1, N2, NROWS, CU_WAVES_K, MINW, true, false, 0, 0, false, float, float, 0, true>;
    p.chunk_prefix = a.d_chunk_prefix;
  }
  int strx_which = -1;
  if constexpr (W4 && (N1 == 32 || N1 == 64) && N2 == 16) {
    if (a.stretch && (pre || a.in_i16) && !a.in_f64 && a.dl_K == 0 && !mf && a.d_chunk_prefix && in_lds && rsg && !a.d_stat_part) {
      using I = int16_t;
      str_used = true;
      kern = a.in_i16 ? (pre ? stft_wave_kernel<N1, N2, NROWS, CU_WAVES_K, MINW, true, true, 0, 0, true, I, float, 0, true>
                             : stft_wave_kernel<N1, N2, NROWS, CU_WAVES_K, MINW, true, false, 0, 0, true, I, float, 0, true>)
                      : stft_wave_kernel<N1, N2, NROWS, CU_WAVES_K, MINW, true, true, 0, 0, true, float, float, 0, true>;
      p.chunk_prefix = a.d_chunk_prefix;
      strx_which = a.in_i16 ? (pre ? 38 : 37) : 36;
    }
  }
  if (a.d_stat_part) {
    if (!str_used || !in_lds || walk == 0 || G::GROUPS != 4 || (rsg && MINW > 2)) {
      set_error("stft_cmvn_batch: not served for this plan and call (needs a 16-lane power-of-two geometry, a segment "
                "walk with its tables and the waves' sums in LDS, float32 samples, no fused pre-emphasis)");
      return PDS_ERR_INVALID;
    }
    p.stat_part = a.d_stat_part;
  }
  int f64_which = -1;
  if (a.in_f64) {
    constexpr bool F64IN = fast_f64in_kind(N1 * N2);
    if constexpr (F64IN) {
      if (!in_lds || (a.out_f64 && pre)) {
        set_error("stft_batch_f64in: not served for this plan (filter table outside LDS, or float64 features with fused pre-emphasis)");
        return PDS_ERR_INVALID;
      }
      mf = false;
      p.win_half = ft.d_win_half;
      p.tw_seed = (const float2 *)ft.d_tw_seed;
      if (a.out_f64)
        kern = rsg ? stft_wave_kernel<N1, N2, NROWS, F64_WAVES, F64_MINW, true, false, false, 0, W4, double, double>
                   : stft_wave_kernel<N1, N2, NROWS, F64_WAVES, F64_MINW, true, false, false, 0, false, double, double>;
      else if (pre)
        kern = rsg ? stft_wave_kernel<N1, N2, NROWS, F64_WAVES, F64_MINW, true, true, false, 0, W4, double, float>
                   : stft_wave_kernel<N1, N2, NROWS, F64_WAVES, F64_MINW, true, true, false, 0, false, double, float>;
      else
        kern = rsg ? stft_wave_kernel<N1, N2, NROWS, F64_WAVES, F64_MINW, true, false, false, 0, W4, double, float>
                   : stft_wave_kernel<N1, N2, NROWS, F64_WAVES, F64_MINW, true, false, false, 0, false, double, float>;
      f64_which = 12 + (a.out_f64 ? 4 : pre ? 2 : 0) + (rsg ? 1 : 0);
    } else {
      set_error("stft_batch_f64in: no fused float64-input kernel for this transform size");
      return PDS_ERR_INVALID;
    }
  }
  int i16_which = -1;
  if (a.in_i16 && a.dl_K == 0 && strx_which < 0) {
    constexpr bool I16IN = fast_f64in_kind(N1 * N2);
    if constexpr (I16IN) {
      if (a.in_f64 || a.out_f64 || a.d_stat_part) {
        set_error("stft_batch_i16in: float32 features, no fused CMVN sums");
        return PDS_ERR_INVALID;
      }
      mf = false;
      kern = pre ? (rsg ? stft_wave_kernel<N1, N2, NROWS, CU_WAVES_K, MINW, true, true, false, 0, W4, int16_t, float>
                        : stft_wave_kernel<N1, N2, NROWS, CU_WAVES_K, MINW, true, true, false, 0, false, int16_t, float>)
                 : (rsg ? stft_wave_kernel<N1, N2, NROWS, CU_WAVES_K, MINW, true, false, false, 0, W4, int16_t, float>
                        : stft_wave_kernel<N1, N2, NROWS, CU_WAVES_K, MINW, true, false, false, 0, false, int16_t, float>);
      i16_which = 32 + (pre ? 2 : 0) + (rsg ? 1 : 0);
    } else {
      set_error("stft_batch_i16in: no fused int16-input kernel for this transform size");
      return PDS_ERR_INVALID;
    }
  }
  int dl_which = -1;
  if (a.dl_K > 0) {
    constexpr bool DELTAS = fast_deltas_kind(N1 * N2) && G::GROUPS == 4;
    if constexpr (DELTAS) {
      const int staged = ((a.dl_K + 1) * (plan->d.num_filts + (plan->d.include_energy ? 1 : 0)) + 3) / 4 * 16 + 64;
      if (!in_lds || !rsg || !dl || ft.rsn_rounds > 2 || (plan->d.include_energy && ft.rs_eslot < 0) || a.out_f64 ||
          staged > G::EXCH_F2 * 2) {
        set_error("stft_deltas_batch: not served for this plan and call (needs the row-segment filter walk with at "
                  "most two rounds in LDS and float32 features)");
        return PDS_ERR_INVALID;
      }
      mf = false;
      using D = double;
      using I = int16_t;
      kern = a.in_f64 ? (pre ? stft_wave_kernel<N1, N2, NROWS, 4 * DMINW, DMINW, true, true, false, 0, true, D, float, 2>
                             : stft_wave_kernel<N1, N2, NROWS, 4 * DMINW, DMINW, true, false, false, 0, true, D, float, 2>)
             : a.in_i16 ? (pre ? stft_wave_kernel<N1, N2, NROWS, 4 * DMINW, DMINW, true, true, false, 0, true, I, float, 2>
                               : stft_wave_kernel<N1, N2, NROWS, 4 * DMINW, DMINW, true, false, false, 0, true, I, float, 2>)
                      : (pre ? stft_wave_kernel<N1, N2, NROWS, 4 * DMINW, DMINW, true, true, false, 0, true, float, float, 2>
                             : stft_wave_kernel<N1, N2, NROWS, 4 * DMINW, DMINW, true, false, false, 0, true, float, float, 2>);
      if (a.in_f64 || PDS_DLT_CHAIN) {
        p.win_half = ft.d_win_half;
        p.tw_seed = (const float2 *)ft.d_tw_seed;
      }
      p.dl_order = a.dl_K;
      dl_which = a.in_i16 ? (pre ? 26 : 21) : 18 + (a.in_f64 ? 1 : 0) + (pre ? 10 : 0);
      for (int j = 0; j < 5; ++j) p.dl_f1[j] = (float)a.dl_taps[j];
      for (int j = 0; j < 9; ++j) p.dl_f2[j] = a.dl_K > 1 ? (float)a.dl_taps[5 + j] : 0.0f;
      p.dl_inner = plan->d.num_filts + (plan->d.include_energy ? 1 : 0);
      p.dl_eslot = plan->d.include_energy ? ft.rs_eslot : -1;
      p.chunk_prefix = a.d_chunk_prefix;
#if defined(PDS_DL_DEBUG_SWITCH) && PDS_DL_DEBUG_SWITCH
      p.dl_debug = std::getenv("PDS_DL_DEBUG") ? std::atoi(std::getenv("PDS_DL_DEBUG")) : 0;
#else
      p.dl_debug = 0;
#endif
    } else {
      set_error("stft_deltas_batch: no fused kernel for this transform size");
      return PDS_ERR_INVALID;
    }
  }
  constexpr int kDevices = 64;
  static std::atomic<size_t> attr_smem[kDevices][40];
  const int which = strx_which >= 0  ? strx_which
                    : dl_which >= 0    ? dl_which
                    : f64_which >= 0 ? f64_which
                    : i16_which >= 0 ? i16_which
                    : pf_used        ? (rsg ? 27 : mseg ? 30 : 31)
                    : str_used       ? 22 + (rsg ? 0 : mseg ? 1 : seg ? 2 : 3)
                    : mseg           ? 20
                                     : (pre ? (rsg ? 5 : 2) : rsg ? 4 : seg ? 3 : (in_lds ? 1 : 0)) + (mf ? 6 : 0);
  const bool cached = plan->device >= 0 && plan->device < kDevices;
  if (!cached || smem > attr_smem[plan->device][which].load(std::memory_order_relaxed)) {
    PDS_HIP(hipFuncSetAttribute((const void *)kern, hipFuncAttributeMaxDynamicSharedMemorySize,
                                (int)smem));
    if (cached) attr_smem[plan->device][which].store(smem, std::memory_order_relaxed);
  }
  int64_t grid = (int64_t)ft.num_cus * wgs_per_cu;
  const int64_t need = (chunks * a.B + waves - 1) / waves;
  if (grid > need) grid = need;
  const int64_t grid_waves = grid * waves;
  p.step_utts = (int)(grid_waves / chunks);
  p.step_chunks = (int)(grid_waves % chunks);
  if (a.dl_K > 0 || str_used) {
    grid = std::min<int64_t>((int64_t)ft.num_cus * wgs_per_cu, std::max<int64_t>(1, (chunks * a.B + 4 * waves - 1) / (4 * waves)));
    if (!a.prefix_prepared) {
      const int32_t rc_prefix = launch_chunk_prefix(a.d_nframes, a.B, G::GROUPS, a.d_chunk_prefix, a.stream);
      if (rc_prefix != PDS_OK) return rc_prefix;
    }
  }
  if (a.grid_waves_out) *a.grid_waves_out = (int32_t)(grid * waves);
  hipLaunchKernelGGL(kern, dim3((unsigned)grid), dim3(waves * 64), smem, a.stream, p);
  PDS_HIP(hipGetLastError());
  return PDS_OK;
}

}
```

Baseline: 4.046 billion.

## Prebuild contiguous LDS table images and per-lane constant blob for kernel prologue

The host now builds, per filter walk, one contiguous image holding the special twiddles, the decoded metadata records and the filter weights. The kernel prologue fills LDS with a single float4 copy loop instead of decoding metadata and copying tables separately. Per-lane window and twiddle constants are packed into an interleaved float4 blob so each lane loads them with vector loads. The first image chunk is loaded early and per-utterance and stretch setup are hoisted ahead of the barrier to overlap prologue latency. This adds device memory per plan, and the f64-output case needs its own image.

```diff
diff --git a/pydrobert-speech_amd/csrc/pds_internal.h b/pydrobert-speech_amd/csrc/pds_internal.h
--- a/pydrobert-speech_amd/csrc/pds_internal.h
+++ b/pydrobert-speech_amd/csrc/pds_internal.h
@@ -26,7 +26,10 @@
   int num_cus = 0;
   float *d_window = nullptr;
   float *d_twiddle = nullptr;
+  float *d_lane_const = nullptr;
   float *d_tw_special = nullptr;
+  float *d_img_ell = nullptr, *d_img_seg = nullptr, *d_img_rs = nullptr, *d_img_rs64 = nullptr, *d_img_rsn = nullptr,
+        *d_img_ms = nullptr;
   float *d_win_half = nullptr;
   float *d_tw_seed = nullptr;
   float *d_ell_w = nullptr;
diff --git a/pydrobert-speech_amd/csrc/stft_fast.hip b/pydrobert-speech_amd/csrc/stft_fast.hip
--- a/pydrobert-speech_amd/csrc/stft_fast.hip
+++ b/pydrobert-speech_amd/csrc/stft_fast.hip
@@ -158,6 +158,33 @@
       tw[((size_t)r * cols + k1) * 2 + 0] = (float)(scale * std::cos(ang));
       tw[((size_t)r * cols + k1) * 2 + 1] = (float)(scale * std::sin(ang));
     }
+  std::vector<float> tws((size_t)n2 * 2);
+  for (int r = 0; r < n2; ++r) {
+    const double ang = -2.0 * M_PI * (double)r / (double)(2 * n2);
+    tws[2 * r] = (float)std::cos(ang);
+    tws[2 * r + 1] = (float)std::sin(ang);
+  }
+  auto lds_image = [&](float **dst, int walk, const int32_t *meta, size_t meta_ints, int tout_bytes, const float *w, size_t wfloats) -> int32_t {
+    const size_t pad = (size_t)walk_meta_pad(walk, (int)meta_ints, n2);
+    std::vector<float> img(((size_t)2 * n2 + pad + wfloats + 3) / 4 * 4, 0.0f);
+    std::copy(tws.begin(), tws.end(), img.begin());
+    float *at = img.data() + 2 * n2;
+    if (walk == 2) {
+      const float one = 1.0f, zero = 0.0f;
+      for (size_t i = 0; i < meta_ints; ++i) {
+        const int32_t m = meta[i], f = (m >> 16) - 1;
+        const int32_t first = (m & 0x3fff) * 16, col = f >= 0 ? ((d.include_energy ? 1 : 0) + f) * tout_bytes : -1;
+        std::memcpy(at + 4 * i, &first, 4);
+        std::memcpy(at + 4 * i + 1, (m & (1 << 14)) ? &one : &zero, 4);
+        std::memcpy(at + 4 * i + 2, (m & (1 << 15)) ? &one : &zero, 4);
+        std::memcpy(at + 4 * i + 3, &col, 4);
+      }
+    } else if (meta_ints) {
+      std::memcpy(at, meta, meta_ints * 4);
+    }
+    if (wfloats) std::copy(w, w + wfloats, at + pad);
+    return upload(dst, img.data(), img.size());
+  };
   std::vector<int32_t> order(d.num_filts);
   for (int f = 0; f < d.num_filts; ++f) order[f] = f;
   auto span = [&](int f) {
@@ -289,6 +316,7 @@
         ft.seg_meta_ints = (int)seg_meta.size();
         if (rc == PDS_OK) rc = upload(&ft.d_seg_w, seg_w.data(), seg_w.size());
         if (rc == PDS_OK) rc = upload(&ft.d_seg_meta, seg_meta.data(), seg_meta.size());
+        if (rc == PDS_OK) rc = lds_image(&ft.d_img_seg, 1, seg_meta.data(), seg_meta.size(), 4, seg_w.data(), seg_w.size());
       }
     }
   }
@@ -311,9 +339,12 @@
           if ((rn.meta[at] >> 16) == 0) ft.rs_eslot = (int)at;
         rc = upload(&ft.d_rsn_w, rn.w.data(), rn.w.size());
         if (rc == PDS_OK) rc = upload(&ft.d_rsn_meta, rn.meta.data(), rn.meta.size());
+        if (rc == PDS_OK) rc = lds_image(&ft.d_img_rsn, 2, rn.meta.data(), (size_t)rn.rounds * 64, 4, rn.w.data(), rn.w.size());
       }
       if (rc == PDS_OK) rc = upload(&ft.d_rs_w, rs.w.data(), rs.w.size());
       if (rc == PDS_OK) rc = upload(&ft.d_rs_meta, rs.meta.data(), rs.meta.size());
+      if (rc == PDS_OK) rc = lds_image(&ft.d_img_rs, 2, rs.meta.data(), (size_t)rs.rounds * 64, 4, rs.w.data(), rs.w.size());
+      if (rc == PDS_OK) rc = lds_image(&ft.d_img_rs64, 2, rs.meta.data(), (size_t)rs.rounds * 64, 8, rs.w.data(), rs.w.size());
     }
   }
   if (n2 == 16 && pow2 && rc == PDS_OK && dense_bank) {
@@ -329,6 +360,7 @@
       ft.ms_reads = ms.reads_per_lane();
       rc = upload(&ft.d_ms_w, ms.w.data(), ms.w.size());
       if (rc == PDS_OK) rc = upload(&ft.d_ms_meta, ms.meta.data(), ms.meta.size());
+      if (rc == PDS_OK) rc = lds_image(&ft.d_img_ms, 3, ms.meta.data(), ms.meta.size(), 4, ms.w.data(), ms.w.size());
     }
   }
   {
@@ -351,10 +383,21 @@
   }
   if (rc == PDS_OK) rc = upload(&ft.d_ell_w, ell_w.data(), ell_w.size());
   if (rc == PDS_OK) rc = upload(&ft.d_ell_meta, ell_meta.data(), ell_meta.size());
+  if (rc == PDS_OK) rc = lds_image(&ft.d_img_ell, 0, ell_meta.data(), (size_t)slots * n2, 4, ell_w.data(), ell_w.size());
   if (rc == PDS_OK) rc = upload(&ft.d_ell_len, ell_len.data(), ell_len.size());
   if (rc == PDS_OK) rc = upload(&ft.d_ell_woff, ell_woff.data(), ell_woff.size());
   if (rc == PDS_OK) rc = upload(&ft.d_window, win.data(), win.size());
   if (rc == PDS_OK) rc = upload(&ft.d_twiddle, tw.data(), tw.size());
+  {
+    const int lcf = lane_const_floats(n1), lcw = lane_const_win_floats(n1);
+    std::vector<float> lc((size_t)n2 * lcf, 0.0f);
+    auto at = [&](int r, int u) -> float & { return lc[((size_t)(u / 4) * n2 + r) * 4 + u % 4]; };
+    for (int r = 0; r < n2; ++r) {
+      for (int k = 0; k < n1; ++k) at(r, k) = win[(size_t)r * n1 + k];
+      for (int k = 0; k < 2 * cols; ++k) at(r, lcw + k) = tw[(size_t)r * cols * 2 + k];
+    }
+    if (rc == PDS_OK) rc = upload(&ft.d_lane_const, lc.data(), lc.size());
+  }
   if (((n1 == 32 || n1 == 64) && n2 == 16) || lean_geometry(n1, n2)) {
     std::vector<float> wh(win), seed((size_t)n2 * 6);
     for (float &v : wh) v *= PDS_RDFT_DIT ? 1.0f : 0.5f;
@@ -367,12 +410,6 @@
       }
     if (rc == PDS_OK) rc = upload(&ft.d_win_half, wh.data(), wh.size());
     if (rc == PDS_OK) rc = upload(&ft.d_tw_seed, seed.data(), seed.size());
-  }
-  std::vector<float> tws((size_t)n2 * 2);
-  for (int r = 0; r < n2; ++r) {
-    const double ang = -2.0 * M_PI * (double)r / (double)(2 * n2);
-    tws[2 * r] = (float)std::cos(ang);
-    tws[2 * r + 1] = (float)std::sin(ang);
   }
   if (rc == PDS_OK) rc = upload(&ft.d_tw_special, tws.data(), tws.size());
   {
@@ -415,6 +452,8 @@
   FastTables &ft = plan->fast;
   (void)hipFree(ft.d_window);
   (void)hipFree(ft.d_twiddle);
+  (void)hipFree(ft.d_lane_const);
+  for (float *img : {ft.d_img_ell, ft.d_img_seg, ft.d_img_rs, ft.d_img_rs64, ft.d_img_rsn, ft.d_img_ms}) (void)hipFree(img);
   (void)hipFree(ft.d_tw_special);
   (void)hipFree(ft.d_win_half);
   (void)hipFree(ft.d_tw_seed);
diff --git a/pydrobert-speech_amd/csrc/stft_wave_kernel.h b/pydrobert-speech_amd/csrc/stft_wave_kernel.h
--- a/pydrobert-speech_amd/csrc/stft_wave_kernel.h
+++ b/pydrobert-speech_amd/csrc/stft_wave_kernel.h
@@ -27,6 +27,7 @@
   int64_t out_stride;
   const float *win_lane;
   const float2 *tw_lane;
+  const float *lane_const;
   const float2 *tw_special;
   const float *win_half;
   const float2 *tw_seed;
@@ -35,6 +36,8 @@
   const int32_t *ell_len;
   const int32_t *ell_woff;
   int ell_wfloats, ell_slots, ell_meta_pad, ell_meta_ints;
+  const float *lds_img;
+  int lds_img4;
   int seg_rounds, seg_len, num_filts;
   int L, S, pad_left, include_energy, use_power, use_log;
   float log_floor, inv_L, preemph;
@@ -118,6 +121,9 @@
   return (PDS_TWOPASS && n1 == 64 && n2 == 16) ? 2688 : lean_geometry(n1, n2) ? groups * cols * (n2 + 4) : one_pass;
 }
 constexpr int win_table_stride(int rows) { return ((rows + 3) & ~3) % 8 == 4 ? ((rows + 3) & ~3) : ((rows + 3) & ~3) + 4; }
+constexpr int walk_meta_pad(int walk, int ints, int n2) { return walk == 2 ? ints * 4 : ((ints > 4 * n2 ? ints : 4 * n2) + 3) / 4 * 4; }
+constexpr int lane_const_win_floats(int n1) { return (n1 + 3) & ~3; }
+constexpr int lane_const_floats(int n1) { return lane_const_win_floats(n1) + ((2 * ((n1 - 1) / 2 + 1) + 3) & ~3); }
 
 template <int N1, int N2, int NROWS>
 struct WaveGeom {
@@ -208,122 +214,7 @@
   constexpr bool WINUSE = G::LEAN || (N1 == 64 && N2 == 16 && (SEG == 2 || PDS_LEAN_1024));
   constexpr int WSTR = win_table_stride(NROWS);
   [[maybe_unused]] float *win_lds = ellw_lds + (ELL_LDS ? p.ell_wfloats : 0);
-  if constexpr (WINLDS || WINUSE) {
-    const float *wsrc = TWCHAIN ? p.win_half : p.win_lane;
-    for (int i = threadIdx.x; i < N2 * WSTR; i += p.waves * 64) {
-      const int rr = i / WSTR, k = i - rr * WSTR;
-      win_lds[i] = k < NROWS ? wsrc[rr * N1 + k] : 0.0f;
-    }
-  }
-  if (threadIdx.x < N2) sw_lds[threadIdx.x] = p.tw_special[threadIdx.x];
   constexpr bool DYN = PDS_DYN && !STRETCH && !PF;
-  [[maybe_unused]] int *ticket_lds = reinterpret_cast<int *>(smem + p.lds_ticket_off);
-  if constexpr (DYN) {
-    if (threadIdx.x == 0) *ticket_lds = p.waves;
-  }
-  if constexpr (STR && G::GROUPS == 4 && (SEG != 0 || (RSG && MINW <= 2))) {
-    if (p.stat_part) {
-      double *z = reinterpret_cast<double *>(smem + p.lds_stat_off);
-      for (int i = threadIdx.x; i < p.waves * 2 * p.stat_cs; i += p.waves * 64) z[i] = 0.0;
-    }
-  }
-  if constexpr (RSG) {
-    int4 *rec_lds = reinterpret_cast<int4 *>(meta_lds);
-    for (int i = threadIdx.x; i < p.seg_rounds * 64; i += nthreads) {
-      const int m = p.ell_meta[i], f = (m >> 16) - 1;
-      rec_lds[i] = make_int4((m & 0x3fff) * 16, __float_as_int((m & (1 << 14)) ? 1.0f : 0.0f),
-                             __float_as_int((m & (1 << 15)) ? 1.0f : 0.0f),
-                             f >= 0 ? ((p.include_energy ? 1 : 0) + f) * (int)sizeof(TOUT) : -1);
-    }
-  } else {
-    for (int i = threadIdx.x; i < p.ell_meta_pad; i += nthreads)
-      meta_lds[i] = i < p.ell_meta_ints ? p.ell_meta[i] : 0;
-  }
-#if PDS_FAST_PROLOGUE
-  static_assert((G::EXCH_F2 * 2) % 4 == 0, "wave areas are zeroed 16 bytes at a time");
-  if constexpr (ELL_LDS) {
-    const float4 *src4 = reinterpret_cast<const float4 *>(p.ell_w);
-    float4 *dst4 = reinterpret_cast<float4 *>(ellw_lds);
-    for (int i = threadIdx.x; i < (p.ell_wfloats >> 2); i += nthreads) dst4[i] = src4[i];
-  }
-  {
-    float4 *z4 = reinterpret_cast<float4 *>(smem);
-    for (int i = threadIdx.x; i < p.waves * (p.area_f / 4); i += nthreads) z4[i] = make_float4(0.0f, 0.0f, 0.0f, 0.0f);
-  }
-#else
-  if constexpr (ELL_LDS)
-    for (int i = threadIdx.x; i < p.ell_wfloats; i += nthreads) ellw_lds[i] = p.ell_w[i];
-  for (int i = threadIdx.x; i < p.waves * p.area_f; i += nthreads) smem[i] = 0.0f;
-#endif
-  __syncthreads();
-
-  [[maybe_unused]] float win[(MF || WINLDS || WINUSE) ? 1 : NROWS];
-  [[maybe_unused]] float twr[(MF || TWCHAIN) ? 1 : COLS], twi[(MF || TWCHAIN) ? 1 : COLS];
-  [[maybe_unused]] float sd[6] = {0.0f, 0.0f, 0.0f, 0.0f, 0.0f, 0.0f};
-  [[maybe_unused]] float mwin[MSLOTS], mare[MF + 1], maim[MF + 1], mtwr[4], mtwi[4];
-  [[maybe_unused]] unsigned moff[MSLOTS];
-  if constexpr (MF > 0) {
-    const float *tab = p.mf_tab;
-#pragma unroll
-    for (int sl = 0; sl < MSLOTS; ++sl) {
-      mwin[sl] = tab[sl * 64 + lane];
-      moff[sl] = (unsigned)reinterpret_cast<const int *>(tab)[(MSLOTS + sl) * 64 + lane] * 4u;
-    }
-#pragma unroll
-    for (int t = 0; t <= MF; ++t) {
-      mare[t] = tab[(3 * MSLOTS + t) * 64 + lane];
-      maim[t] = tab[(3 * MSLOTS + MF + 1 + t) * 64 + lane];
-    }
-#pragma unroll
-    for (int v = 0; v < 4; ++v) {
-      const float2 t = reinterpret_cast<const float2 *>(tab + (3 * MSLOTS + 2 * (MF + 1)) * 64)[v * 64 + lane];
-      mtwr[v] = t.x;
-      mtwi[v] = t.y;
-    }
-  } else {
-    if constexpr (!WINLDS && !WINUSE) {
-      const float *wsrc = TWCHAIN ? p.win_half : p.win_lane;
-#pragma unroll
-      for (int n1 = 0; n1 < NROWS; ++n1) win[n1] = wsrc[rho * N1 + n1];
-    }
-    if constexpr (TWCHAIN) {
-#pragma unroll
-      for (int j = 0; j < 3; ++j) {
-        const float2 t = p.tw_seed[rho * 3 + j];
-        sd[2 * j] = t.x;
-        sd[2 * j + 1] = t.y;
-      }
-    } else {
-#pragma unroll
-      for (int k1 = 1; k1 <= NREG; ++k1) {
-        const float2 t = p.tw_lane[rho * COLS + k1];
-        twr[k1] = t.x;
-        twi[k1] = t.y;
-      }
-    }
-  }
-  [[maybe_unused]] float pfv[PF ? NROWS : 1];
-  [[maybe_unused]] float wl[WINLDS ? NROWS : 1];
-  [[maybe_unused]] auto read_window = [&]() {
-    if constexpr (WINLDS) {
-      const float4 *w4 = reinterpret_cast<const float4 *>(win_lds + rho * WSTR);
-#pragma unroll
-      for (int j = 0; j < (NROWS + 3) / 4; ++j) {
-        const float4 w = w4[j];
-        const float wv[4] = {w.x, w.y, w.z, w.w};
-#pragma unroll
-        for (int u = 0; u < 4; ++u)
-          if (4 * j + u < NROWS) wl[4 * j + u] = wv[u];
-      }
-    }
-  };
-  read_window();
-  [[maybe_unused]] bool pf_ready = false;
-  [[maybe_unused]] const int pf_lane = __mul24(g, p.S) + r;
-  const int L = p.L, S = p.S;
-  const bool use_power = p.use_power != 0;
-  const int col0 = p.include_energy ? 1 : 0;
-
   int b = 0;
   int wg = blockIdx.x;
 #ifndef PDS_NO_XCD_MAP
@@ -343,6 +234,158 @@
       ++rb;
     }
   }
+  const float4 *img_src = reinterpret_cast<const float4 *>(p.lds_img);
+  float4 *img_dst = reinterpret_cast<float4 *>(sw_lds);
+  const float4 img_first = img_src[(int)threadIdx.x < p.lds_img4 ? threadIdx.x : 0];
+
+  constexpr bool BLOB = MF == 0 && !TWCHAIN && !WINLDS && !WINUSE;
+  [[maybe_unused]] float win[(MF || WINLDS || WINUSE) ? 1 : NROWS];
+  [[maybe_unused]] float twr[(MF || TWCHAIN) ? 1 : COLS], twi[(MF || TWCHAIN) ? 1 : COLS];
+  [[maybe_unused]] float sd[6] = {0.0f, 0.0f, 0.0f, 0.0f, 0.0f, 0.0f};
+  [[maybe_unused]] float mwin[MSLOTS], mare[MF + 1], maim[MF + 1], mtwr[4], mtwi[4];
+  [[maybe_unused]] unsigned moff[MSLOTS];
+  if constexpr (MF > 0) {
+    const float *tab = p.mf_tab;
+#pragma unroll
+    for (int sl = 0; sl < MSLOTS; ++sl) {
+      mwin[sl] = tab[sl * 64 + lane];
+      moff[sl] = (unsigned)reinterpret_cast<const int *>(tab)[(MSLOTS + sl) * 64 + lane] * 4u;
+    }
+#pragma unroll
+    for (int t = 0; t <= MF; ++t) {
+      mare[t] = tab[(3 * MSLOTS + t) * 64 + lane];
+      maim[t] = tab[(3 * MSLOTS + MF + 1 + t) * 64 + lane];
+    }
+#pragma unroll
+    for (int v = 0; v < 4; ++v) {
+      const float2 t = reinterpret_cast<const float2 *>(tab + (3 * MSLOTS + 2 * (MF + 1)) * 64)[v * 64 + lane];
+      mtwr[v] = t.x;
+      mtwi[v] = t.y;
+    }
+  } else if constexpr (BLOB) {
+    const float4 *blob = reinterpret_cast<const float4 *>(p.lane_const) + rho;
+#pragma unroll
+    for (int j = 0; j < (NROWS + 3) / 4; ++j) {
+      const float4 w = blob[j * N2];
+      const float wv[4] = {w.x, w.y, w.z, w.w};
+#pragma unroll
+      for (int u = 0; u < 4; ++u)
+        if (4 * j + u < NROWS) win[4 * j + u] = wv[u];
+    }
+#pragma unroll
+    for (int j = 0; j < (COLS + 1) / 2; ++j) {
+      const float4 t = blob[(lane_const_win_floats(N1) / 4 + j) * N2];
+      twr[2 * j] = t.x;
+      twi[2 * j] = t.y;
+      if (2 * j + 1 < COLS) {
+        twr[2 * j + 1] = t.z;
+        twi[2 * j + 1] = t.w;
+      }
+    }
+  } else {
+    if constexpr (!WINLDS && !WINUSE) {
+      const float *wsrc = TWCHAIN ? p.win_half : p.win_lane;
+#pragma unroll
+      for (int n1 = 0; n1 < NROWS; ++n1) win[n1] = wsrc[rho * N1 + n1];
+    }
+    if constexpr (TWCHAIN) {
+#pragma unroll
+      for (int j = 0; j < 3; ++j) {
+        const float2 t = p.tw_seed[rho * 3 + j];
+        sd[2 * j] = t.x;
+        sd[2 * j + 1] = t.y;
+      }
+    } else {
+#pragma unroll
+      for (int k1 = 1; k1 <= NREG; ++k1) {
+        const float2 t = p.tw_lane[rho * COLS + k1];
+        twr[k1] = t.x;
+        twi[k1] = t.y;
+      }
+    }
+  }
+  int nfr = 0, n = 0;
+  int64_t sig_off = 0, out_row = 0;
+  if (!STRETCH && b < p.num_utts) {
+    nfr = (int)load_const(p.nframes + b);
+    n = (int)load_const(p.lengths + b);
+    sig_off = load_const(p.offsets + b);
+    out_row = load_const(p.row_off + b);
+  }
+
+  [[maybe_unused]] int left = 0, e_lo = 0, e_hi = 0, c_last = -1;
+  if constexpr (STRETCH) {
+    const int gw = wg * p.waves + wave, GW = (int)gridDim.x * p.waves;
+    const int total = (int)load_const(p.chunk_prefix + p.num_utts);
+    const int per = total / GW, rem = total - per * GW;
+    const int pos = gw * per + (gw < rem ? gw : rem);
+    left = per + (gw < rem ? 1 : 0);
+    int lo = 0, hi = p.num_utts;
+    while (left > 0 && hi - lo > 1) {
+      const int mid = (lo + hi) >> 1;
+      if ((int)load_const(p.chunk_prefix + mid) <= pos) lo = mid; else hi = mid;
+    }
+    b = lo;
+    e_lo = left > 0 ? pos - (int)load_const(p.chunk_prefix + lo) : 0;
+    chunk = 0;
+  }
+  if constexpr (WINLDS || WINUSE) {
+    const float *wsrc = TWCHAIN ? p.win_half : p.win_lane;
+    for (int i = threadIdx.x; i < N2 * WSTR; i += p.waves * 64) {
+      const int rr = i / WSTR, k = i - rr * WSTR;
+      win_lds[i] = k < NROWS ? wsrc[rr * N1 + k] : 0.0f;
+    }
+  }
+  [[maybe_unused]] int *ticket_lds = reinterpret_cast<int *>(smem + p.lds_ticket_off);
+  if constexpr (DYN) {
+    if (threadIdx.x == 0) *ticket_lds = p.waves;
+  }
+  if constexpr (STR && G::GROUPS == 4 && (SEG != 0 || (RSG && MINW <= 2))) {
+    if (p.stat_part) {
+      double *z = reinterpret_cast<double *>(smem + p.lds_stat_off);
+      for (int i = threadIdx.x; i < p.waves * 2 * p.stat_cs; i += p.waves * 64) z[i] = 0.0;
+    }
+  }
+  if (threadIdx.x < p.lds_img4) img_dst[threadIdx.x] = img_first;
+  for (int i = threadIdx.x + nthreads; i < p.lds_img4; i += nthreads) img_dst[i] = img_src[i];
+  keep_alive(img_first.x);
+  keep_alive(img_first.y);
+  keep_alive(img_first.z);
+  keep_alive(img_first.w);
+#if PDS_FAST_PROLOGUE
+  static_assert((G::EXCH_F2 * 2) % 4 == 0, "wave areas are zeroed 16 bytes at a time");
+  {
+    float4 *z4 = reinterpret_cast<float4 *>(smem);
+    for (int i = threadIdx.x; i < p.waves * (p.area_f / 4); i += nthreads) z4[i] = make_float4(0.0f, 0.0f, 0.0f, 0.0f);
+  }
+#else
+  for (int i = threadIdx.x; i < p.waves * p.area_f; i += nthreads) smem[i] = 0.0f;
+#endif
+  __syncthreads();
+  [[maybe_unused]] const unsigned long long st_bar = PDS_STAMPS ? __builtin_readcyclecounter() : 0;
+
+  [[maybe_unused]] float pfv[PF ? NROWS : 1];
+  [[maybe_unused]] float wl[WINLDS ? NROWS : 1];
+  [[maybe_unused]] auto read_window = [&]() {
+    if constexpr (WINLDS) {
+      const float4 *w4 = reinterpret_cast<const float4 *>(win_lds + rho * WSTR);
+#pragma unroll
+      for (int j = 0; j < (NROWS + 3) / 4; ++j) {
+        const float4 w = w4[j];
+        const float wv[4] = {w.x, w.y, w.z, w.w};
+#pragma unroll
+        for (int u = 0; u < 4; ++u)
+          if (4 * j + u < NROWS) wl[4 * j + u] = wv[u];
+      }
+    }
+  };
+  read_window();
+  [[maybe_unused]] bool pf_ready = false;
+  [[maybe_unused]] const int pf_lane = __mul24(g, p.S) + r;
+  const int L = p.L, S = p.S;
+  const bool use_power = p.use_power != 0;
+  const int col0 = p.include_energy ? 1 : 0;
+
   [[maybe_unused]] auto take_ticket = [&](const int t) {
     const int jn = (int)__umulhi((unsigned)t, p.waves_rcp), o = t - jn * p.waves;
     while (rnd < jn && rb < p.num_utts) {
@@ -374,32 +417,10 @@
     sig_off_ = load_const(p.offsets + pb_);
     out_row_ = load_const(p.row_off + pb_);
   };
-  int nfr = 0, n = 0;
-  int64_t sig_off = 0, out_row = 0;
-  if (!STRETCH && b < p.num_utts) {
-    nfr = (int)load_const(p.nframes + b);
-    n = (int)load_const(p.lengths + b);
-    sig_off = load_const(p.offsets + b);
-    out_row = load_const(p.row_off + b);
-  }
   constexpr int DR = 2;
-  [[maybe_unused]] int left = 0, e_lo = 0, e_hi = 0, c_last = -1;
   [[maybe_unused]] bool piece_open = false, ran = false;
   [[maybe_unused]] float Wp[DR][4], Wc[DR][4], e_keep = 0.0f;
   if constexpr (STRETCH) {
-    const int gw = wg * p.waves + wave, GW = (int)gridDim.x * p.waves;
-    const int total = (int)load_const(p.chunk_prefix + p.num_utts);
-    const int per = total / GW, rem = total - per * GW;
-    const int pos = gw * per + (gw < rem ? gw : rem);
-    left = per + (gw < rem ? 1 : 0);
-    int lo = 0, hi = p.num_utts;
-    while (left > 0 && hi - lo > 1) {
-      const int mid = (lo + hi) >> 1;
-      if ((int)load_const(p.chunk_prefix + mid) <= pos) lo = mid; else hi = mid;
-    }
-    b = lo;
-    e_lo = left > 0 ? pos - (int)load_const(p.chunk_prefix + lo) : 0;
-    chunk = 0;
 #pragma unroll
     for (int rd = 0; rd < DR; ++rd)
 #pragma unroll
@@ -478,6 +499,7 @@
   [[maybe_unused]] unsigned long long st_acc[8] = {0, 0, 0, 0, 0, 0, 0, 0};
   [[maybe_unused]] unsigned long long st_prev = PDS_STAMPS ? __builtin_readcyclecounter() : 0;
   [[maybe_unused]] const unsigned long long st_loop = st_prev;
+  [[maybe_unused]] unsigned long long st_first[2] = {0, 0};
   while (STRETCH || b < p.num_utts) {
     if constexpr (STRETCH) {
       if (!piece_open) {
@@ -555,7 +577,10 @@
       continue;
     }
     PDS_STAMP(7, 0);
-    if constexpr (PDS_STAMPS != 0) ++st_acc[6];
+    if constexpr (PDS_STAMPS != 0) {
+      if (PDS_STAMPS == 1 && st_acc[6] == 1) st_first[1] = st_prev;
+      ++st_acc[6];
+    }
     PDS_PHASE(0);
     [[maybe_unused]] int nfr_nx = 0, n_nx = 0;
     [[maybe_unused]] int64_t sig_off_nx = 0, out_row_nx = 0;
@@ -669,6 +694,9 @@
       }
       PDS_STAMP(0, 0);
       PDS_STAMP(1, 1);
+      if constexpr (PDS_STAMPS == 1) {
+        if (st_acc[6] == 1) st_first[0] = st_prev;
+      }
       PDS_PHASE(4);
       float sv[4][MF], dv[4][MF], cv[4], uv[4];
 #pragma unroll
@@ -911,6 +939,9 @@
       }
       PDS_STAMP(0, 0);
       PDS_STAMP(1, 1);
+      if constexpr (PDS_STAMPS == 1) {
+        if (st_acc[6] == 1) st_first[0] = st_prev;
+      }
       PDS_PHASE(4);
       if constexpr (WINLDS) {
 #pragma unroll
@@ -1652,12 +1683,16 @@
   }
   if constexpr (PDS_STAMPS) {
     if (p.stamps && lane == 0) {
-      unsigned long long *dst = p.stamps + ((size_t)blockIdx.x * p.waves + wave) * 12;
+      unsigned long long *dst = p.stamps + ((size_t)blockIdx.x * p.waves + wave) * 16;
 #pragma unroll
       for (int i = 0; i < 8; ++i) dst[i] = st_acc[i];
+      const unsigned long long st_end = __builtin_readcyclecounter();
       dst[8] = st_entry;
       dst[9] = st_loop;
-      dst[10] = __builtin_readcyclecounter();
+      dst[10] = st_end;
+      dst[11] = st_bar;
+      dst[12] = st_first[0];
+      dst[13] = st_first[1] ? st_first[1] : st_end;
     }
   }
 }
diff --git a/pydrobert-speech_amd/csrc/stft_wave_launch.h b/pydrobert-speech_amd/csrc/stft_wave_launch.h
--- a/pydrobert-speech_amd/csrc/stft_wave_launch.h
+++ b/pydrobert-speech_amd/csrc/stft_wave_launch.h
@@ -30,6 +30,7 @@
   p.out_stride = a.out_stride;
   p.win_lane = ft.d_window;
   p.tw_lane = (const float2 *)ft.d_twiddle;
+  p.lane_const = ft.d_lane_const;
   p.tw_special = (const float2 *)ft.d_tw_special;
   constexpr bool LEAN_ALL = G::LEAN || (PDS_LEAN_1024 && N1 == 64 && N2 == 16);
   p.win_half = LEAN_ALL ? ft.d_win_half : nullptr;
@@ -100,7 +101,7 @@
     if (cand == 3 && (!MSG || ft.ms_rounds == 0 || pre || a.in_f64 || a.in_i16)) continue;
     if ((cand == 2 && !dl && ft.rs_rounds == 0) || (cand == 1 && (ft.seg_rounds == 0 || pre || a.in_f64 || a.in_i16))) continue;
     const int meta_ints = cand == 3 ? ft.ms_meta_ints : cand == 2 ? (dl ? ft.rsn_rounds : ft.rs_rounds) * 64 : cand == 1 ? ft.seg_meta_ints : ft.ell_slots * N2;
-    const int meta_pad = cand == 2 ? meta_ints * 4 : (std::max(meta_ints, USLOTS * N2) + 3) / 4 * 4;
+    const int meta_pad = walk_meta_pad(cand, meta_ints, N2);
     const size_t fixed = (size_t)N2 * 8 + (size_t)meta_pad * 4 + (cand == 2 && pf_ok ? pf_extra : 0) + lean_extra +
                          (cand == 3 && MSEG3 ? mseg3_extra : 0);
     const size_t table_bytes = (size_t)(cand == 3 ? ft.ms_wfloats : cand == 2 ? (dl ? ft.rsn_wfloats : ft.rs_wfloats) : cand == 1 ? ft.seg_wfloats : ft.ell_wfloats) * 4;
@@ -162,6 +163,15 @@
     }
     return launch_stft_generic_f32(plan, a);
   }
+  p.lds_img = walk == 3   ? ft.d_img_ms
+              : walk == 1 ? ft.d_img_seg
+              : walk == 2 ? (dl ? ft.d_img_rsn : (a.in_f64 && a.out_f64) ? ft.d_img_rs64 : ft.d_img_rs)
+                          : ft.d_img_ell;
+  p.lds_img4 = (2 * N2 + p.ell_meta_pad + (in_lds ? p.ell_wfloats : 0)) / 4;
+  if (!p.lds_img) {
+    set_error("stft_batch: the plan has no table image for this filter walk");
+    return PDS_ERR_INVALID;
+  }
   p.preemph = (float)a.preemph;
   p.preemph_d = a.preemph;
   p.waves = waves;
```

Result: no change. 4.070 billion (median of 6 runs) (+0.6%).
